# justinmgarrigus/accel-sim-framework-distributed

Measured on AMD Instinct MI355X. Metric: sim KIPS (whole node), higher is better.
Workload: dtype n/a (integer cycle-level model)

## Files before the change

build_native.py:

```python
#!/usr/bin/env python3
from __future__ import annotations

import argparse
import os
import shutil
import subprocess
import sys
import sysconfig

ROOT = os.path.dirname(os.path.abspath(__file__))
PKG = os.path.join(ROOT, "accel_sim_framework_distributed_amd")
ROCM = os.environ.get("ROCM_PATH", "/opt/rocm")
BINARY_PATH_APPS = ("nw", "lud", "hotspot", "backprop", "devcalls")
ARCH = os.environ.get("PYTORCH_ROCM_ARCH", "gfx950")

CORE_SRC = [
    "csrc/config/options.cc",
    "csrc/config/sim_options.cc",
    "csrc/config/icnt_config.cc",
    "csrc/trace/trace.cc",
    "csrc/engine/cpu_engine.cc",
    "csrc/engine/check_engine.cc",
    "csrc/power/power.cc",
    "csrc/power/arch_energy.cc",
    "csrc/driver/simulator.cc",
    "csrc/driver/dump.cc",
    "csrc/driver/debugger.cc",
    "csrc/driver/icnt_bench.cc",
    "csrc/parallel/linksim.cc",
]
HIP_SRC = ["csrc/engine/gpu_engine.hip", "csrc/engine/engine_k_lds.hip", "csrc/engine/engine_k_prof.hip",
           "csrc/engine/engine_k_global.hip", "csrc/engine/engine_k_split.hip", "csrc/engine/engine_k_split2.hip", "csrc/engine/ingest_mfma.hip",
           "csrc/engine/lane_check.hip", "csrc/engine/icnt_sweep.hip"]
STUB_SRC = ["csrc/engine/gpu_stub.cc"]


def _pybind_includes():
    import pybind11
    return [pybind11.get_include(), sysconfig.get_paths()["include"]]


def ext_suffix():
    return sysconfig.get_config_var("EXT_SUFFIX") or ".so"


def have_hipcc():
    return shutil.which("hipcc") is not None or os.path.exists(os.path.join(ROCM, "bin", "hipcc"))


def write_ninja(cpu_only: bool, extra_targets: bool) -> str:
    bdir = os.path.join(ROOT, "build")
    os.makedirs(bdir, exist_ok=True)
    hipcc = shutil.which("hipcc") or os.path.join(ROCM, "bin", "hipcc")
    inc = " ".join(f"-I{p}" for p in [os.path.join(ROOT, "csrc")] + _pybind_includes())
    cxxflags = f"-std=c++17 -O3 -g -fPIC -fopenmp -pthread -Wall -Wno-unused-variable -Wno-unused-function {inc}"
    hipflags = (f"-std=c++17 -O3 -fPIC --offload-arch={ARCH} -munsafe-fp-atomics "
                f"-I{os.path.join(ROOT, 'csrc')}")
    ldflags = f"-fopenmp -pthread -L{ROCM}/lib -Wl,-rpath,{ROCM}/lib"
    lines = [
        "ninja_required_version = 1.3",
        f"cxxflags = {cxxflags}",
        f"hipflags = {hipflags}",
        f"ldflags = {ldflags}",
        "rule cxx",
        "  command = g++ $cxxflags -MMD -MF $out.d -c $in -o $out",
        "  depfile = $out.d",
        "  deps = gcc",
        "  description = CXX $in",
        "rule hip",
        f"  command = {hipcc} $hipflags -MMD -MF $out.d -c $in -o $out",
        "  depfile = $out.d",
        "  deps = gcc",
        "  description = HIP $in",
        "rule link_so",
        "  command = g++ -shared $in -o $out $ldflags $libs",
        "  description = LINK $out",
        "rule link_exe",
        "  command = g++ $in -o $out $ldflags $libs",
        "  description = LINK $out",
        "rule hipexe",
        f"  command = {hipcc} $hipflags $in -o $out $libs",
        "rule isatrace",
        f"  command = {sys.executable} {os.path.join(PKG, 'isatrace', 'build.py')} $in -o $out \"--libs=$libs\" -- "
        f"-munsafe-fp-atomics -fPIC -I{os.path.join(ROOT, 'csrc')}",
        "  description = HIPEXE $out",
        "rule isatrace_bin",
        f"  command = {sys.executable} {os.path.join(PKG, 'isatrace', 'build.py')} $src -o $out --device-from $in "
        f"\"--libs=$libs\" -- -munsafe-fp-atomics -fPIC -I{os.path.join(ROOT, 'csrc')}",
        "  description = HIPEXE-BIN $out",
    ]
    objs = []
    for s in CORE_SRC:
        o = os.path.join(bdir, s.replace("/", "_") + ".o")
        lines.append(f"build {o}: cxx {os.path.join(ROOT, s)}")
        objs.append(o)
    gpu_objs = []
    if not cpu_only:
        for s in HIP_SRC:
            o = os.path.join(bdir, s.replace("/", "_") + ".o")
            lines.append(f"build {o}: hip {os.path.join(ROOT, s)}")
            gpu_objs.append(o)
        libs = "-lamdhip64"
    else:
        for s in STUB_SRC:
            o = os.path.join(bdir, s.replace("/", "_") + ".o")
            lines.append(f"build {o}: cxx {os.path.join(ROOT, s)}")
            gpu_objs.append(o)
        libs = ""
    bind_o = os.path.join(bdir, "bindings.o")
    lines.append(f"build {bind_o}: cxx {os.path.join(ROOT, 'csrc/bindings/py_asim.cc')}")
    main_o = os.path.join(bdir, "main.o")
    lines.append(f"build {main_o}: cxx {os.path.join(ROOT, 'csrc/driver/main.cc')}")
    so = os.path.join(PKG, "_asim" + ext_suffix())
    lines.append(f"build {so}: link_so {' '.join(objs + gpu_objs + [bind_o])}")
    lines.append(f"  libs = {libs}")
# ... 126 lines not shown
```

csrc/bindings/py_asim.cc:

```cpp
#include <chrono>
#include <pybind11/functional.h>
#include <pybind11/numpy.h>
#include <pybind11/pybind11.h>
#include <pybind11/stl.h>

#include <cstring>

#include "../config/icnt_config.h"
#include "../driver/icnt_bench.h"
#include "../driver/simulator.h"
#include "../engine/icnt_sweep.h"

namespace py = pybind11;
using namespace asim;
static const size_t kLinkPktBytes = sizeof(LinkPkt);

namespace {

py::dict link_dict(const LinkParams& p) {
  py::dict d;
  d["link_gbps"] = p.link_gbps;
  d["latency_ns"] = p.latency_ns;
  d["links"] = p.links;
  d["slice_bytes"] = p.slice_bytes;
// ... 533 lines not shown
            if (space != "shared" && space != "global") throw py::value_error("space is 'shared' or 'global'" + at);
            const uint64_t width = py::cast<uint64_t>(t[1]);
            if (width > 255) throw py::value_error("width above 255 bytes per lane" + at);
            const std::string op = py::cast<std::string>(t[4]);
            TInst in{};
            in.cls = OC_LOAD;
            in.space = space == "shared" ? S_SHARED : S_GLOBAL;
            in.width = (uint8_t)width;
            in.mask = py::cast<uint64_t>(t[2]);
            if (!op.empty()) in.opcode = decode_opcode(op, 950).opcode;
            TMem m{};
            if (py::isinstance<py::tuple>(t[3])) {
              const py::tuple bs = py::cast<py::tuple>(t[3]);
              if (bs.size() != 2) throw py::value_error("(base, stride) expected" + at);
              const py::int_ stride = py::cast<py::int_>(bs[1]);
              const long long sv = PyLong_AsLongLong(stride.ptr());
              if (PyErr_Occurred()) {
                PyErr_Clear();
                throw py::value_error("stride outside int32" + at);
              }
              if (sv < INT32_MIN || sv > INT32_MAX) throw py::value_error("stride outside int32" + at);
              m.base = py::cast<uint64_t>(bs[0]);
              m.stride = (int32_t)sv;
              m.list = kNoMem;
            } else {
              const std::vector<uint64_t> a = py::cast<std::vector<uint64_t>>(t[3]);
              if ((size_t)__builtin_popcountll(in.mask) != a.size())
                throw py::value_error("one address per active lane" + at);
              m.list = (uint32_t)k.addrs.size();
              k.addrs.insert(k.addrs.end(), a.begin(), a.end());
              m.base = a.empty() ? 0 : a[0];
            }
            in.mem = (uint32_t)k.mems.size();
            k.mems.push_back(m);
            k.insts.push_back(in);
          }
          k.streams.push_back(WStream{0, (uint32_t)k.insts.size()});
          auto results = [](const ReadyKernel& r) {
            py::list out;
            for (const TInst& in : r.insts) {
              py::list acc;
              if (in.mem != kNoMem)
                for (uint32_t q = 0; q < in.width; ++q) {
                  const TAcc& a = r.accs.at((size_t)in.mem + q);
                  acc.append(py::make_tuple(a.line, (int)a.sectors, (int)a.bytes, (int)a.bank));
                }
              out.append(py::make_tuple(in.space == S_SHARED ? "shared" : "global", (int)in.width, acc));
            }
            return out;
          };
          py::dict d;
          d["host"] = results(coalesce_kernel(k, c));
          d["ran"] = false;
          if (device < 0) return d;
          IngestStats st;
          std::vector<uint8_t> where;
          st.on_device = &where;
          ReadyKernel g;
          if (!gpu_coalesce_kernel(k, c, device, g, &st)) return d;
          d["ran"] = true;
          d["device"] = results(g);
          py::list w;
          for (uint8_t v : where) w.append((int)v);
          d["on_device"] = w;
          d["smem_device"] = st.smem_jobs;
          d["smem_host"] = st.smem_host;
          d["gmem_device"] = st.gmem_jobs;
          d["gmem_host"] = st.gmem_host;
          d["mfma"] = st.mfma;
          return d;
        },
        py::arg("insts"), py::arg("args"), py::arg("device") = -1);
  m.def("lane_policy_check",
        [](const std::string& name, int n, const std::vector<uint64_t>& values, const std::vector<uint64_t>& mask) {
          LaneCheckResult r = lane_policy_check(name, n, values, mask);
          py::dict d;
          d["ran"] = r.ran;
          d["seq"] = r.seq;
          d["stat_words"] = r.stat_words;
          auto bytes_of = [](const std::vector<uint64_t>& v) {
            return py::bytes(reinterpret_cast<const char*>(v.data()), v.size() * 8);
          };
          if (!r.seq_state.empty()) d["seq_state"] = bytes_of(r.seq_state);
          if (r.ran) {
            d["wave"] = r.wave;
            d["stray"] = r.stray;
            if (!r.wave_state.empty()) d["wave_state"] = bytes_of(r.wave_state);
          }
          return d;
        },
        py::arg("case"), py::arg("n"), py::arg("values"), py::arg("mask"));
  m.def("stream_compare", [](const std::string& path, const std::vector<std::string>& args, uint32_t step) {
    SimCfg c = cfg_from_args(args);
    ReadyKernel w = coalesce_kernel(load_kernel_text(path), c);
    ReadyKernel r = open_streamed_kernel(path, c);
    const uint32_t wpc = w.warps_per_cta;
    int64_t bad_cta = -1;
    step = std::max<uint32_t>(1, step);
    for (uint32_t lo = 0; lo < w.n_cta && bad_cta < 0; lo += step) {
      const uint32_t hi = std::min(w.n_cta, lo + step);
      r.resident(lo, hi);
      for (uint32_t cta = lo; cta < hi && bad_cta < 0; ++cta)
        for (uint32_t wi = 0; wi < wpc && bad_cta < 0; ++wi) {
          const WStream& a = w.streams[(size_t)cta * wpc + wi];
          const WStream& b = r.streams[(size_t)(cta - r.cta_lo) * wpc + wi];
          if (a.count != b.count) bad_cta = cta;
          for (uint32_t j = 0; j < a.count && bad_cta < 0; ++j) {
            TInst x = w.insts[a.begin + j];
            TInst y = r.insts[((b.begin + j) - (r.ibase & kStreamInstMask)) & kStreamInstMask];
            const uint32_t xm = x.mem, ym = y.mem;
            x.mem = y.mem = 0;
            if (memcmp(&x, &y, sizeof(TInst)) != 0 || (xm == kNoMem) != (ym == kNoMem)) {
              bad_cta = cta;
              break;
            }
            if (xm == kNoMem) continue;
            const uint64_t yl = (ym - (r.abase & kStreamAccMask)) & kStreamAccMask;
            for (uint32_t q = 0; q < x.width && bad_cta < 0; ++q)
              if (memcmp(&w.accs[xm + q], &r.accs[yl + q], sizeof(TAcc)) != 0) bad_cta = cta;
          }
        }
    }
    py::dict d;
    d["equal"] = bad_cta < 0;
    d["bad_cta"] = bad_cta;
    d["whole_bytes"] = w.host_bytes();
    d["stream_peak_bytes"] = r.host_peak_bytes;
    d["n_cta"] = w.n_cta;
    return d;
  });
  m.def("coalesce_summary", [](const std::string& path, const std::vector<std::string>& args) {
    SimCfg c = cfg_from_args(args);
    ReadyKernel r = coalesce_kernel(load_kernel(path), c);
    py::dict d;
    d["n_accs"] = (uint64_t)r.accs.size();
    uint64_t mem = 0, shared_deg = 0, nshared = 0;
    for (auto& in : r.insts) {
      if (in.mem != kNoMem) mem++;
      if ((in.cls == OC_LOAD || in.cls == OC_STORE) && in.space == S_SHARED) {
        nshared++;
        shared_deg += in.width;
      }
    }
    d["mem_insts"] = mem;
    d["shared_insts"] = nshared;
    d["shared_degree_sum"] = shared_deg;
    py::list acc;
    for (size_t i = 0; i < r.accs.size() && i < 4096; ++i)
      acc.append(py::make_tuple(r.accs[i].line, r.accs[i].sectors, r.accs[i].bytes));
    d["accs"] = acc;
    return d;
  });

  py::class_<Simulator>(m, "Simulator")
      .def(py::init([](const std::vector<std::string>& args, bool echo) {
             py::gil_scoped_release nogil;
             auto* s = new Simulator(args);
             s->set_echo(echo);
             return s;
           }),
           py::arg("args"), py::arg("echo") = false)
      .def("run", &Simulator::run, py::call_guard<py::gil_scoped_release>())
      .def("run_command", &Simulator::run_command, py::call_guard<py::gil_scoped_release>())
      .def("num_commands", [](Simulator& s) { return s.commands().size(); })
      .def("load_commands", &Simulator::load_commands, py::call_guard<py::gil_scoped_release>())
      .def("print_header", [](Simulator& s) { s.load_commands(); })
// ... 171 lines not shown
```

csrc/engine/engine.h:

```cpp
#pragma once
#include <cstring>
#include <memory>
#include <stdexcept>
#include <map>
#include <string>
#include <vector>

#include "../model/epoch.h"
#include "../power/power_eval.h"
#include "../trace/trace.h"

namespace asim {

struct RunLimits {
  uint64_t max_cycle = 0;
  uint64_t max_epochs = 0;
};

struct PwrArm {
  PwrCoef coef;
  uint64_t freq = 0;
  uint64_t t_prev = 0;
  double s_prev[PS_COUNT] = {};
  uint32_t n_sm = 0;
// ... 61 lines not shown
    for (int r = 0; r < PR_COUNT; ++r) {
      const int j = pwr_sum_of(r);
      if (j >= 0) S[j] += (double)pwr_raw_sm(*sm[i], r);
    }
  for (size_t i = 0; i < nmem; ++i)
    for (int r = 0; r < PR_COUNT; ++r) {
      const int j = pwr_sum_of(r);
      if (j >= 0) S[j] += (double)pwr_raw_mem(*mem[i], r);
    }
}

inline PwrSample pwr_take(PwrArm& a, const double* S, uint64_t now) {
  PwrSample o{};
  double d[PS_COUNT];
  for (int j = 0; j < PS_COUNT; ++j) d[j] = S[j] - a.s_prev[j];
  pwr_activity(d, now > a.t_prev ? (double)(now - a.t_prev) : 1.0, a.n_sm, o);
  pwr_power(a.coef, a.coef.coef, a.n_sm, 1.0, 1.0, 1.0, o);
  o.now = now;
  for (int j = 0; j < PS_COUNT; ++j) a.s_prev[j] = S[j];
  a.t_prev = now;
  return o;
}

inline uint32_t backlog_cap(const SimCfg& c) {
  uint64_t b = (uint64_t)c.n_sm * c.icnt_out_limit;
  return (uint32_t)(b < 16384 ? b : 16384);
}

struct EngineStateHeader {
  uint64_t magic = 0x41534d5354415445ull;
  uint64_t version = 8;
  uint64_t n_sm = 0, n_mem = 0, sm_bytes = 0, ch_bytes = 0, pub_bytes = 0;
  uint64_t box_req = 0, cnt_req = 0, box_rep = 0, cnt_rep = 0;
  uint64_t ovf = 0;
  uint64_t mall = 0;
  uint64_t links = 0;
  uint64_t cycle = 0, epoch = 0, ready = 0;
};

struct StateOut {
  std::vector<uint8_t>& v;
  void put(const void* p, size_t n) {
    const size_t o = v.size();
    v.resize(o + n);
    if (n) memcpy(v.data() + o, p, n);
  }
};
struct StateIn {
  const std::vector<uint8_t>& v;
  size_t off = 0;
  const uint8_t* take(size_t n) {
    if (off + n > v.size()) throw std::runtime_error("engine state: truncated image");
    const uint8_t* p = v.data() + off;
    off += n;
    return p;
  }
  void get(void* dst, size_t n) { memcpy(dst, take(n), n); }
};
void check_state_header(const EngineStateHeader& h, const EngineStateHeader& want);

std::unique_ptr<Engine> make_cpu_engine();
std::unique_ptr<Engine> make_gpu_engine();
bool gpu_engine_available();
std::unique_ptr<Engine> make_check_engine(std::unique_ptr<Engine> primary, std::unique_ptr<Engine> reference,
                                          uint64_t interval, uint64_t corrupt_at = 0, bool corrupt_mailbox = false);
int gpu_cu_count();
int gpu_cus_per_sim(uint32_t n_sm, uint32_t n_mem);
std::map<std::string, uint64_t> gpu_pool_stats();
void gpu_pool_trim();
void* gpu_pool_alloc(size_t bytes);
void gpu_pool_release(void* p);
std::map<std::string, uint64_t> gpu_batch_stats();
std::map<std::string, std::map<std::string, uint64_t>> gpu_engine_modes();
struct EngineKernelInfo {
  int num_regs = 0, local_bytes = 0, shared_static = 0, max_threads = 0, binary_version = 0;
  size_t lds_dynamic = 0, sm_state_bytes = 0, chan_state_bytes = 0;
  bool valid = false;
};
EngineKernelInfo gpu_engine_kernel_info();

struct LaneCheckResult {
  std::vector<uint64_t> seq, wave;
  std::vector<uint64_t> seq_state, wave_state;
  bool ran = false;
  bool stray = false;
  uint32_t stat_words = (uint32_t)kStatWords;
};
LaneCheckResult lane_policy_check(const std::string& name, int n, const std::vector<uint64_t>& values,
                                  const std::vector<uint64_t>& mask);

inline uint64_t mall_lines(const SimCfg& c) { return (uint64_t)c.mall_sets * c.mall_assoc; }

uint32_t reply_cap(const SimCfg& c);
void check_core_clock(const SimCfg& c, uint64_t per_core);
void host_memcpy_fill(ChanState* chs, uint32_t nch, const SimCfg& c, uint64_t addr, uint64_t bytes);
void host_flush_l2(ChanState* chs, uint32_t nch, const SimCfg& c, bool writeback = false, L2Line* mall = nullptr);
void init_sm_state(SMState& s, uint32_t id);
void init_chan_state(ChanState& ch, uint32_t id, const SimCfg& c);

}
```

csrc/engine/engine_k_global.hip:

```cpp
#include "engine_kernel.h"

namespace asim {

template __global__ void engine_kernel<WavePar, true, kModeGlobal>(GpuArgs);

__global__ void ASIM_ENGINE_KERNEL_ATTRS engine_batch_kernel(const GpuArgs* __restrict__ jobs,
                                                             const uint16_t* __restrict__ block_job) {
  const uint32_t j = block_job[blockIdx.x];
  const GpuArgs a = jobs[j];
  engine_body<WavePar, true, kModeGlobal>(a, blockIdx.x - a.block0);
}

ASIM_ENGINE_CFG_UPLOAD(global)

}
```

csrc/engine/engine_k_lds.hip:

```cpp
#include "engine_kernel.h"

namespace asim {

template __global__ void engine_kernel<WavePar, false, kModeLds>(GpuArgs);
template __global__ void engine_kernel<WavePar, true, kModeLds>(GpuArgs);

ASIM_ENGINE_CFG_UPLOAD(lds)

}
```

csrc/engine/engine_k_prof.hip:

```cpp
#include "engine_kernel.h"

namespace asim {

template __global__ void engine_kernel<WaveParProf, false, kModeLds>(GpuArgs);
template __global__ void engine_kernel<WaveParProf, true, kModeLds>(GpuArgs);
template __global__ void engine_kernel<WaveParProf, true, kModeGlobal>(GpuArgs);
template __global__ void engine_kernel<WaveParProf, true, kModeSplit>(GpuArgs);

ASIM_ENGINE_CFG_UPLOAD(prof)

}
```

csrc/engine/engine_k_split.hip:

```cpp
#include "engine_kernel.h"

namespace asim {

template __global__ void engine_kernel<WavePar, true, kModeSplit>(GpuArgs);

__global__ void ASIM_ENGINE_KERNEL_ATTRS engine_batch_split_kernel(const GpuArgs* __restrict__ jobs,
                                                                   const uint16_t* __restrict__ block_job) {
  const uint32_t j = block_job[blockIdx.x];
  const GpuArgs a = jobs[j];
  engine_body<WavePar, true, kModeSplit>(a, blockIdx.x - a.block0);
}

ASIM_ENGINE_CFG_UPLOAD(split)

}
```

csrc/engine/engine_k_split2.hip:

```cpp
#include "engine_kernel.h"

namespace asim {

#define ASIM_SPLIT2_KERNEL_ATTRS __launch_bounds__(64) __attribute__((amdgpu_waves_per_eu(2, 2)))

__global__ void ASIM_SPLIT2_KERNEL_ATTRS engine_split2_kernel(GpuArgs a) {
  engine_body<WavePar, true, kModeSplit>(a, blockIdx.x);
}

ASIM_ENGINE_CFG_UPLOAD(split2)

}
```

csrc/engine/engine_kernel.h:

```cpp
#pragma once
#include <hip/hip_runtime.h>

#include "../model/icnt_router_par.h"
#include "engine.h"
#include "grid_barrier.h"
#include "wave_par.h"
#include "sm_split.h"

namespace asim {

constexpr int kCfgSlots = 64;
static __constant__ SimCfg g_cfg[kCfgSlots];

struct PwrDev {
  PwrCoef coef;
  uint64_t freq;
  uint64_t t_prev;
  uint64_t next;
  uint32_t n_sm;
  uint32_t n;
  uint32_t cap;
  uint32_t pad;
  double s_prev[kPwrSumPad];
  double* rows;
// ... 109 lines not shown
template <class T>
__device__ __forceinline__ T* as_global(T* p) {
  typedef __attribute__((address_space(1))) T gT;
  return (T*)(gT*)p;
}

struct WaveParProf : WavePar {
  static __device__ __forceinline__ void prof(int k) {
    ProfLds* p = reinterpret_cast<ProfLds*>(g_lds + kProfOff);
    uint64_t t = __builtin_amdgcn_s_memtime();
    if ((threadIdx.x & 63) == 0) {
      p->acc[p->slot] += t - p->last;
      p->slot = (uint32_t)k;
      p->last = t;
    }
    __builtin_amdgcn_wave_barrier();
  }
  static __device__ __forceinline__ void tick(int k) {
    ProfLds* p = reinterpret_cast<ProfLds*>(g_lds + kProfOff);
    if ((threadIdx.x & 63) == 0) p->acc[k] += 1;
    __builtin_amdgcn_wave_barrier();
  }
};

typedef double f64x4 __attribute__((ext_vector_type(4)));

__device__ __forceinline__ void pwr_row_sm(double* row, const SMStats& st) {
  for (int k = (int)(threadIdx.x & 63); k < kPwrRawPad; k += 64) row[k] = k < PR_COUNT ? (double)pwr_raw_sm(st, k) : 0.0;
}
__device__ __forceinline__ void pwr_row_ch(double* row, const ChanState& ch, uint32_t nsub) {
  for (int k = (int)(threadIdx.x & 63); k < kPwrRawPad; k += 64) {
    double v = 0;
    if (k < PR_COUNT)
      for (uint32_t j = 0; j < nsub; ++j) v += (double)pwr_raw_mem(ch.sp[j].st, k);
    row[k] = v;
  }
}

__device__ void pwr_evaluate(PwrDev& pw, uint32_t nunits, uint64_t now) {
  const int lane = (int)(threadIdx.x & 63);
  constexpr int kCt = kPwrSumPad / 16;
  f64x4 acc[kCt];
#pragma unroll
  for (int ct = 0; ct < kCt; ++ct) acc[ct] = f64x4{0.0, 0.0, 0.0, 0.0};
  const double* rows = pw.rows;
  for (uint32_t t = 0; t < (nunits + 15u) / 16u; ++t) {
    const uint32_t u = 16u * t + (uint32_t)(lane & 15);
    for (int k4 = 0; k4 < kPwrRawPad / 4; ++k4) {
      const int k = 4 * k4 + (lane >> 4);
      const double av = u < nunits ? rows[(size_t)u * kPwrRawPad + k] : 0.0;
      const int sj = k < PR_COUNT ? pwr_sum_of(k) : -1;
#pragma unroll
      for (int ct = 0; ct < kCt; ++ct) {
        const double bv = sj == 16 * ct + (lane & 15) ? 1.0 : 0.0;
        acc[ct] = __builtin_amdgcn_mfma_f64_16x16x4f64(av, bv, acc[ct], 0, 0, 0);
      }
    }
  }
  double* S = reinterpret_cast<double*>(g_lds + kPwrOff);
  double* D = S + kPwrSumPad;
#pragma unroll
  for (int ct = 0; ct < kCt; ++ct) {
    double v = acc[ct][0] + acc[ct][1] + acc[ct][2] + acc[ct][3];
    v += __shfl_xor(v, 16);
    v += __shfl_xor(v, 32);
    if (lane < 16) S[16 * ct + lane] = v;
  }
  __syncthreads();
  if (lane < PS_COUNT) D[lane] = S[lane] - pw.s_prev[lane];
  __syncthreads();
  if (lane == 0) {
    const uint32_t i = pw.n < pw.cap ? pw.n : pw.cap - 1;
    PwrSample& o = pw.ring[i];
    pwr_activity(D, now > pw.t_prev ? (double)(now - pw.t_prev) : 1.0, pw.n_sm, o);
    pwr_power(pw.coef, pw.coef.coef, pw.n_sm, 1.0, 1.0, 1.0, o);
    o.now = now;
    pw.t_prev = now;
    pw.n = pw.n + 1;
  }
  if (lane < PS_COUNT) pw.s_prev[lane] = S[lane];
  __syncthreads();
}

template <class P, bool kSliced, int kMode>
__device__ __forceinline__ void engine_body(const GpuArgs& a, const uint32_t b) {
  constexpr bool kGlobal = kMode == kModeGlobal, kSplit = kMode == kModeSplit;
  const SimCfg& c = g_cfg[a.cfg_slot];
  const uint64_t E = c.icnt_latency;
  SMState* s = reinterpret_cast<SMState*>(g_lds + kStateOff);
  ChanState* ch = reinterpret_cast<ChanState*>(g_lds + kStateOff);
  const uint32_t nunits = c.n_sm + c.n_mem;
  const uint32_t nsmb = a.nblocks - a.ch_blocks;
  auto unit_k = [&](uint32_t k) -> uint32_t {
    if (!a.ch_blocks) return b + k * a.nblocks;
    return b < nsmb ? b + k * nsmb : c.n_sm + (b - nsmb) + k * a.ch_blocks;
  };
  const uint32_t nmine = !kSliced ? 1u
                         : !a.ch_blocks ? (nunits - 1 - b) / a.nblocks + 1
                         : b < nsmb ? (c.n_sm - 1 - b) / nsmb + 1
                                    : (c.n_mem - 1 - (b - nsmb)) / a.ch_blocks + 1;
  const uint32_t u0 = unit_k(0);
  uint32_t loaded = u0;
  auto bind = [&](uint32_t u) {
    if (u < c.n_sm) s = as_global(&a.sms[u]);
    else ch = as_global(&a.chs[u - c.n_sm]);
  };
  uint32_t hot = u0;
  auto swap_to = [&](uint32_t u) {
    if (kGlobal) {
      bind(u);
      loaded = u;
      return;
    }
    if (kSplit) {
      loaded = u;
      if (u >= c.n_sm) {
        ch = as_global(&a.chs[u - c.n_sm]);
        return;
      }
      if (u == hot) return;
      if (hot < c.n_sm) copy_bytes(&a.sms[hot], s, kSmHotBytes);
      copy_bytes(s, &a.sms[u], kSmHotBytes);
      hot = u;
      return;
    }
    if (!kSliced || u == loaded) return;
    if (loaded < c.n_sm) swap_out(&a.sms[loaded], s);
    else swap_out(&a.chs[loaded - c.n_sm], ch);
    if (u < c.n_sm) swap_in(s, &a.sms[u]);
    else swap_in(ch, &a.chs[u - c.n_sm]);
    loaded = u;
  };
  if (kGlobal)
    bind(u0);
  else if (kSplit && u0 < c.n_sm)
    copy_bytes(s, &a.sms[u0], kSmHotBytes);
  else if (kSplit) {
    hot = ~0u;
    ch = as_global(&a.chs[u0 - c.n_sm]);
  } else if (u0 < c.n_sm)
    copy_state(s, &a.sms[u0]);
  else
    copy_state(ch, &a.chs[u0 - c.n_sm]);
  KernelTab* ktl = reinterpret_cast<KernelTab*>(g_lds + kKtOff);
  {
    static_assert(sizeof(KernelTab) % 16 == 0, "kernel table must be 16-byte granular");
    const uint4* src = reinterpret_cast<const uint4*>(a.kt);
    uint4* dst = reinterpret_cast<uint4*>(ktl);
    for (int i = (int)(threadIdx.x & 63); i < (int)(sizeof(KernelTab) / 16); i += 64) dst[i] = src[i];
  }
  ProfLds* pl = reinterpret_cast<ProfLds*>(g_lds + kProfOff);
  if ((threadIdx.x & 63) == 0) {
    pl->last = __builtin_amdgcn_s_memtime();
    pl->slot = 31;
    for (int i = 0; i < kProfSlots; ++i) pl->acc[i] = 0;
  }
  __syncthreads();
  const KernelTab& kt = *ktl;
  SmCtx sx;
  sx.cfg = &c;
  sx.kt = &kt;
  sx.out_cap = a.cap_req;
  sx.n_src_sm = c.n_sm;
  sx.rt_st = c.link_contention == 2 ? a.link_free : nullptr;
  MemCtx mx;
  mx.cfg = &c;
  mx.out_cap = a.cap_rep;
  mx.n_src_sub = c.n_subpart;
  mx.ovf = a.ovf;
  mx.ovf_cap = a.ovf_cap;
  mx.rt_st = c.link_contention == 2 ? a.link_free : nullptr;
  mx.mall = nullptr;
  uint64_t epoch = a.epoch0, cycle = a.cycle0;
  uint64_t t_work0 = a.ework ? __builtin_amdgcn_s_memtime() : 0;
  uint32_t done = 0, dead = 0, capped = 0;
  uint32_t n = 0;
  uint32_t nbar = 0;
  uint64_t pw_next = a.pw ? a.pw->next : 0;
  bool failed = false;
  uint64_t reqm[2] = {~0ull, ~0ull}, repm[2] = {~0ull, ~0ull};
  for (; n < a.max_epochs;) {
    const uint32_t cur = (uint32_t)(epoch & 1), prev = cur ^ 1u;
    const uint64_t t0 = cycle, t1 = t0 + E;
    uint32_t first_k = 0;
    for (uint32_t k = 0; k < nmine; ++k)
      if (unit_k(k) == loaded) first_k = k;
    for (uint32_t j = 0; j < nmine; ++j) {
      const uint32_t u = unit_k((first_k + j) % nmine);
      swap_to(u);
      if (u < c.n_sm) {
        sx.outbox = a.box_req[cur];
        sx.outcnt = a.cnt_req[cur];
        if constexpr (kSplit) {
          SmSplit sp(*s, *as_global(&a.sms[u]));
          sm_epoch<P>(sp, sx, *a.pub, prev, t0, t1, a.box_rep[prev], a.cnt_rep[prev], a.cap_rep, c.n_subpart, epoch,
                      repm);
          sm_publish<P>(sp, sx, *a.pub, cur);
        } else {
          sm_epoch<P>(*s, sx, *a.pub, prev, t0, t1, a.box_rep[prev], a.cnt_rep[prev], a.cap_rep,
                      c.n_subpart, epoch, repm);
          sm_publish<P>(*s, sx, *a.pub, cur);
        }
      } else {
        mx.outbox = a.box_rep[cur];
        mx.outcnt = a.cnt_rep[cur];
        mx.mall = a.mall ? a.mall + (size_t)(u - c.n_sm) * ((size_t)c.mall_sets * c.mall_assoc) : nullptr;
        mx.win_end = core_fs(c, t1);
        chan_epoch<P>(*ch, mx, a.box_req[prev], a.cnt_req[prev], a.cap_req, core_fs(c, t0), reqm);
        chan_publish<P>(*ch, mx, *a.pub, cur);
      }
    }
    ++n;
    P::prof(26);
    uint64_t t_arrive = 0;
    if (a.ework) {
      t_arrive = __builtin_amdgcn_s_memtime();
      if ((threadIdx.x & 63) == 0) a.ework[b] = (uint32_t)(t_arrive - t_work0);
    }
    uint32_t was_last = 0;
    if (!grid_barrier_b(a.ctl, b, a.nblocks, nbar++, &was_last)) break;
    if (a.link_free) {
      const bool rt_par = c.link_contention == 2 && c.router_pass == 1;
      if (rt_par) {
        if (b < 2) {
          const uint32_t dirs = !a.link_refs2 ? (uint32_t)RT_DIR_BOTH : b == 0 ? (uint32_t)RT_DIR_REQ : (uint32_t)RT_DIR_REP;
          const uint32_t rs = rt_epoch_run_par<P>(c, a.box_req[cur], a.cnt_req[cur], a.cap_req, a.box_rep[cur],
                                                  a.cnt_rep[cur], a.cap_rep, a.link_free,
                                                  b == 0 ? a.link_refs : a.link_refs2, dirs, a.rt_pc);
          if (rs != RT_STATUS_OK && (threadIdx.x & 63) == 0)
            __hip_atomic_store(&a.ctl->error, kCtlErrRouterCap, __ATOMIC_RELAXED, __HIP_MEMORY_SCOPE_AGENT);
        }
      } else if (b == 0) {
        icnt_epoch_pass<P>(c, a.box_req[cur], a.cnt_req[cur], a.cap_req, a.box_rep[cur], a.cnt_rep[cur], a.cap_rep,
                           a.link_free, a.link_refs);
      }
      if (!grid_barrier_b(a.ctl, b, a.nblocks, nbar++)) break;
      if (rt_par && P::uni(__hip_atomic_load(&a.ctl->error, __ATOMIC_RELAXED, __HIP_MEMORY_SCOPE_AGENT))) break;
    }
    P::prof(27);
    if (a.ework) {
      const uint64_t t_exit = __builtin_amdgcn_s_memtime();
      if ((threadIdx.x & 63) == 0 && was_last) { pl->acc[34] += t_exit - t_arrive; pl->acc[35] += 1; }
      if (b == 0) {
        uint64_t mk = 0;
        for (uint32_t j = threadIdx.x & 63; j < a.nblocks; j += 64) {
          const uint64_t k = (uint64_t)a.ework[j] << 32 | j;
          mk = k > mk ? k : mk;
        }
        mk = WavePar::red_max64(mk);
        const uint32_t m = (uint32_t)(mk >> 32);
        if ((threadIdx.x & 63) == 0) {
          pl->acc[32] += m;
          pl->acc[33] += 1;
          atomicAdd((unsigned long long*)&a.prof[(size_t)(uint32_t)mk * kProfSlots + 30], 1ull);
        }
      }
      t_work0 = t_exit;
    }
    const uint64_t mc = a.pw ? (a.max_cycle ? (a.max_cycle < pw_next ? a.max_cycle : pw_next) : pw_next) : a.max_cycle;
    EpochDecision d = epoch_decide<P>(c, *a.pub, cur, t1, kt, epoch, mc);
    reqm[0] = P::uni(d.req_dst[0]);
    reqm[1] = P::uni(d.req_dst[1]);
    repm[0] = P::uni(d.rep_dst[0]);
    repm[1] = P::uni(d.rep_dst[1]);
    P::prof(28);
    ++epoch;
    cycle = P::uni(d.next_start);
    if (a.pw) {
      const bool exits = P::uni(d.done) || P::uni(d.deadlock) || P::uni(d.limit) || (a.max_cycle && cycle >= a.max_cycle);
      if (exits || cycle >= pw_next) {
        for (uint32_t k = 0; k < nmine; ++k) {
          const uint32_t u = unit_k(k);
          double* row = a.pw->rows + (size_t)u * kPwrRawPad;
          if (u < c.n_sm) pwr_row_sm(row, (!kGlobal && u == (kSplit ? hot : loaded)) ? s->st : a.sms[u].st);
          else pwr_row_ch(row, (!kGlobal && !kSplit && u == loaded) ? *ch : a.chs[u - c.n_sm], c.n_sub_per_mem);
        }
        if (!grid_barrier_b(a.ctl, b, a.nblocks, nbar++)) { failed = true; break; }
        if (b == a.nblocks - 1) pwr_evaluate(*a.pw, nunits, cycle);
        pw_next = cycle + a.pw->freq;
      }
    }
    if (P::uni(d.done)) { done = P::uni(d.done); break; }
    if (P::uni(d.deadlock)) { dead = 1; break; }
    if (P::uni(d.limit)) { capped = 1; break; }
    if (P::uni(d.refill)) break;
    if (a.max_cycle && cycle >= a.max_cycle) break;
  }
  P::prof(31);
  if (kGlobal)
    ;
  else if (kSplit) {
    if (hot < c.n_sm) copy_bytes(&a.sms[hot], s, kSmHotBytes);
  } else if (loaded < c.n_sm)
    copy_state(&a.sms[loaded], s);
  else
    copy_state(&a.chs[loaded - c.n_sm], ch);
  if (a.prof && (threadIdx.x & 63) < kProfSlots && (threadIdx.x & 63) != 30) a.prof[(size_t)b * kProfSlots + (threadIdx.x & 63)] += pl->acc[threadIdx.x & 63];
  (void)failed;
  if (a.pw && b == 0 && (threadIdx.x & 63) == 0) a.pw->next = pw_next;
  if (b == 0 && (threadIdx.x & 63) == 0) {
    a.ctl->done = done;
    a.ctl->deadlock = dead;
    a.ctl->cap = capped;
    a.ctl->end_cycle = cycle;
    a.ctl->end_epoch = epoch;
    a.ctl->epochs_run = n;
  }
}


#define ASIM_ENGINE_KERNEL_ATTRS __launch_bounds__(64) __attribute__((amdgpu_waves_per_eu(1, 1)))

template <class P, bool kSliced, int kMode>
__global__ void ASIM_ENGINE_KERNEL_ATTRS engine_kernel(GpuArgs a) {
  engine_body<P, kSliced, kMode>(a, blockIdx.x);
}

__global__ void ASIM_ENGINE_KERNEL_ATTRS engine_batch_kernel(const GpuArgs* __restrict__ jobs,
                                                             const uint16_t* __restrict__ block_job);
__global__ void ASIM_ENGINE_KERNEL_ATTRS engine_batch_split_kernel(const GpuArgs* __restrict__ jobs,
                                                                   const uint16_t* __restrict__ block_job);

__global__ void engine_split2_kernel(GpuArgs a);

#define ASIM_ENGINE_CFG_UPLOAD(name)                                                         \
  hipError_t engine_upload_cfg_##name(const SimCfg& c, int slot) {                          \
    return hipMemcpyToSymbol(HIP_SYMBOL(g_cfg), &c, sizeof(SimCfg), sizeof(SimCfg) * (size_t)slot, \
                             hipMemcpyHostToDevice);                                         \
  }

}
```

csrc/engine/gpu_engine.hip:

```cpp
#include <hip/hip_runtime.h>

#include <algorithm>
#include <cerrno>
#include <csignal>
#include <cstdio>
#include <cstring>
#include <map>
#include <memory>
#include <stdexcept>
#include <string>

#include <fcntl.h>
#include <sys/file.h>
#include <sys/stat.h>
#include <unistd.h>
#include <chrono>
#include <condition_variable>
#include <deque>
#include <mutex>
#include <vector>

#include "engine_kernel.h"
#include "trace_window.h"

namespace asim {

#define HIPCHECK(x)                                                                                  \
  do {                                                                                               \
    hipError_t e_ = (x);                                                                             \
    if (e_ != hipSuccess)                                                                            \
      throw std::runtime_error(std::string("HIP error: ") + hipGetErrorString(e_) + " at " #x);    \
  } while (0)

extern template __global__ void engine_kernel<WavePar, false, kModeLds>(GpuArgs);
extern template __global__ void engine_kernel<WavePar, true, kModeLds>(GpuArgs);
extern template __global__ void engine_kernel<WaveParProf, false, kModeLds>(GpuArgs);
extern template __global__ void engine_kernel<WaveParProf, true, kModeLds>(GpuArgs);
extern template __global__ void engine_kernel<WavePar, true, kModeGlobal>(GpuArgs);
extern template __global__ void engine_kernel<WaveParProf, true, kModeGlobal>(GpuArgs);
extern template __global__ void engine_kernel<WavePar, true, kModeSplit>(GpuArgs);
extern template __global__ void engine_kernel<WaveParProf, true, kModeSplit>(GpuArgs);
hipError_t engine_upload_cfg_lds(const SimCfg& c, int slot);
hipError_t engine_upload_cfg_prof(const SimCfg& c, int slot);
hipError_t engine_upload_cfg_global(const SimCfg& c, int slot);
hipError_t engine_upload_cfg_split(const SimCfg& c, int slot);
hipError_t engine_upload_cfg_split2(const SimCfg& c, int slot);

namespace {

class DeviceCuTable {
 public:
  struct Ent {
    int32_t pid;
    int32_t cus;
  };
  static constexpr int kMax = 256;
  explicit DeviceCuTable(int dev) {
    char bus[64] = {0};
    if (hipDeviceGetPCIBusId(bus, sizeof(bus), dev) != hipSuccess) snprintf(bus, sizeof(bus), "dev%d", dev);
    for (char* q = bus; *q; ++q)
      if (*q == ':' || *q == '.') *q = '_';
    path_ = std::string("/tmp/asim_gpu_cus_") + bus + ".lock";
    fd_ = open(path_.c_str(), O_RDWR | O_CREAT, 0666);
    if (fd_ >= 0) (void)fchmod(fd_, 0666);
  }
  ~DeviceCuTable() {
    if (fd_ >= 0) close(fd_);
  }
  void acquire(int n, int cap) {
    if (fd_ < 0) return;
    for (int spin = 0;; ++spin) {
      if (flock(fd_, LOCK_EX) != 0) return;
      std::vector<Ent> e = load();
      int used = 0;
      for (const Ent& x : e) used += x.cus;
      if (used + n <= cap || e.empty()) {
        e.push_back(Ent{(int32_t)getpid(), (int32_t)n});
        store(e);
        flock(fd_, LOCK_UN);
        return;
      }
      flock(fd_, LOCK_UN);
      usleep(spin < 100 ? 200 : 2000);
    }
  }
  void release(int n) {
    if (fd_ < 0 || flock(fd_, LOCK_EX) != 0) return;
    std::vector<Ent> e = load();
    for (size_t i = 0; i < e.size(); ++i)
      if (e[i].pid == (int32_t)getpid() && e[i].cus == n) {
        e.erase(e.begin() + (long)i);
        break;
      }
    store(e);
    flock(fd_, LOCK_UN);
  }

 private:
  std::vector<Ent> load() {
    std::vector<Ent> e(kMax);
    const ssize_t r = pread(fd_, e.data(), sizeof(Ent) * kMax, 0);
    e.resize(r > 0 ? (size_t)r / sizeof(Ent) : 0);
    std::vector<Ent> live;
    for (const Ent& x : e)
      if (x.pid > 0 && x.cus > 0 && (kill(x.pid, 0) == 0 || errno == EPERM)) live.push_back(x);
    return live;
  }
  void store(const std::vector<Ent>& e) {
    if (ftruncate(fd_, 0) != 0) return;
    if (!e.empty()) (void)pwrite(fd_, e.data(), sizeof(Ent) * e.size(), 0);
  }
  std::string path_;
  int fd_ = -1;
};

constexpr uint32_t kCuSlots = 840;
constexpr uint32_t kMaxBlocksPerCu = 8;
uint32_t block_slots(size_t lds) {
  const size_t per_cu = lds ? (160 * 1024) / lds : kMaxBlocksPerCu;
  return kCuSlots / (uint32_t)std::max<size_t>(1, std::min<size_t>(per_cu, kMaxBlocksPerCu));
}
int gpu_state_mode() {
  const char* e = getenv("ASIM_GPU_STATE");
  if (!e || !*e) return kModeSplit;
  const std::string v(e);
  return v == "global" ? kModeGlobal : v == "lds" ? kModeLds : kModeSplit;
}
bool gpu_state_global() { return gpu_state_mode() == kModeGlobal; }
int split_waves() {
  const char* e = getenv("ASIM_GPU_SPLIT_WAVES");
  return e && atoi(e) == 2 ? 2 : 1;
}
int g_occ_api = 0;
uint32_t mode_blocks_per_cu(int mode) {
  if (mode == kModeLds) return 1;
  static std::mutex mu;
  static uint32_t cache[3] = {0, 0, 0};
  std::lock_guard<std::mutex> g(mu);
  if (!cache[mode]) {
    int occ = 0;
    const void* f = mode == kModeGlobal ? (const void*)engine_batch_kernel
                    : split_waves() == 2 ? (const void*)engine_split2_kernel
                                         : (const void*)engine_kernel<WavePar, true, kModeSplit>;
    const size_t lds = mode == kModeGlobal ? kLdsBytesGlobal : kLdsBytesSplit;
    if (hipOccupancyMaxActiveBlocksPerMultiprocessor(&occ, f, 64, (int)lds) != hipSuccess) occ = 2;
    g_occ_api = occ;
    occ = occ > 1 ? occ - 1 : 1;
    if (const char* e = getenv("ASIM_GPU_BLOCKS_PER_CU"))
      if (atoi(e) > 0) occ = atoi(e);
    cache[mode] = (uint32_t)std::min<int>(occ, (int)kMaxBlocksPerCu);
  }
  return cache[mode];
}
uint32_t global_blocks_per_cu() { return mode_blocks_per_cu(kModeGlobal); }
struct BlockPlan {
  uint32_t nblocks, ch_blocks;
};
BlockPlan block_plan(uint32_t n_sm, uint32_t n_mem, int mode, uint32_t cap) {
  BlockPlan p{n_sm + n_mem, 0};
  if (mode == kModeSplit && n_sm > 0 && n_mem > 0) {
    uint32_t pack = 1;
    if (const char* e = getenv("ASIM_GPU_CH_PER_BLOCK"))
      if (atoi(e) > 0) pack = (uint32_t)atoi(e);
    const uint32_t chb = (n_mem + pack - 1) / pack;
    if (pack > 1 && n_sm + chb <= cap) p = BlockPlan{n_sm + chb, chb};
  }
  if (p.nblocks > cap) p = BlockPlan{cap, 0};
  return p;
}
uint32_t engine_block_slots(int mode) { return kCuSlots / mode_blocks_per_cu(mode); }
bool profiling_env() {
  const char* pe = getenv("ASIM_GPU_PROFILE");
  return pe && *pe && *pe != '0';
}
bool gpu_batch_on() {
  const char* e = getenv("ASIM_GPU_BATCH");
  return e && std::string(e) == "1";
}

class CuPool {
 public:
  static CuPool& get() {
    static CuPool p;
    return p;
  }
  void init(int cus) {
    std::lock_guard<std::mutex> g(mu_);
    if (cap_ == 0) {
      cap_ = free_ = cus;
      int dev = 0;
      if (hipGetDevice(&dev) == hipSuccess) table_.reset(new DeviceCuTable(dev));
    }
  }
  void acquire(int n) {
    {
      std::unique_lock<std::mutex> g(mu_);
      cv_.wait(g, [&] { return free_ >= n; });
      free_ -= n;
    }
    if (table_) table_->acquire(n, cap_);
  }
  void release(int n) {
    if (table_) table_->release(n);
    {
      std::lock_guard<std::mutex> g(mu_);
      free_ += n;
    }
    cv_.notify_all();
  }
  int capacity() {
    std::lock_guard<std::mutex> g(mu_);
    return cap_;
  }

 private:
  std::mutex mu_;
  std::condition_variable cv_;
  int cap_ = 0, free_ = 0;
  std::unique_ptr<DeviceCuTable> table_;
};

class CfgSlots {
 public:
  static CfgSlots& get() {
    static CfgSlots s;
    return s;
// ... 279 lines not shown
      if (e == hipSuccess) e = hipMalloc(&sl.d_bj, sizeof(uint16_t) * nbk);
      if (e == hipSuccess) e = hipHostMalloc(&sl.h_jobs, sizeof(GpuArgs) * nj);
      if (e == hipSuccess) e = hipHostMalloc(&sl.h_bj, sizeof(uint16_t) * nbk);
      if (e != hipSuccess) {
        sl.jobs_cap = sl.blocks_cap = 0;
        return e;
      }
      sl.jobs_cap = nj;
      sl.blocks_cap = nbk;
    }
    uint32_t b0 = 0;
    for (size_t j = 0; j < njobs; ++j) {
      GpuArgs a = take[j]->a;
      a.block0 = b0;
      sl.h_jobs[j] = a;
      for (uint32_t i = 0; i < take[j]->nb; ++i) sl.h_bj[b0 + i] = (uint16_t)j;
      b0 += take[j]->nb;
    }
    hipError_t e = hipMemcpyAsync(sl.d_jobs, sl.h_jobs, sizeof(GpuArgs) * njobs, hipMemcpyHostToDevice, sl.stream);
    if (e == hipSuccess) e = hipMemcpyAsync(sl.d_bj, sl.h_bj, sizeof(uint16_t) * blocks, hipMemcpyHostToDevice, sl.stream);
    for (size_t j = 0; j < njobs && e == hipSuccess; ++j) e = hipMemsetAsync(take[j]->a.ctl, 0, sizeof(GpuCtl), sl.stream);
    if (e != hipSuccess) return e;
    CuPool::get().acquire((int)slots);
    if (mode == kModeSplit)
      hipLaunchKernelGGL(engine_batch_split_kernel, dim3(blocks), dim3(64), kLdsBytesSplit, sl.stream,
                         (const GpuArgs*)sl.d_jobs, (const uint16_t*)sl.d_bj);
    else
      hipLaunchKernelGGL(engine_batch_kernel, dim3(blocks), dim3(64), kLdsBytesGlobal, sl.stream,
                         (const GpuArgs*)sl.d_jobs, (const uint16_t*)sl.d_bj);
    e = hipGetLastError();
    for (size_t j = 0; j < njobs; ++j) {
      const hipError_t ce =
          hipMemcpyAsync(take[j]->h_ctl, take[j]->a.ctl, sizeof(GpuCtl), hipMemcpyDeviceToHost, sl.stream);
      if (e == hipSuccess) e = ce;
    }
    const hipError_t se = hipStreamSynchronize(sl.stream);
    CuPool::get().release((int)slots);
    return e != hipSuccess ? e : se;
  }

  std::mutex mu_;
  std::condition_variable cv_;
  std::deque<Sub*> pending_;
  std::chrono::steady_clock::time_point first_;
  int running_ = 0;
  int in_flight_ = 0;
  int in_run_ = 0;
  Slot slots_[kMaxBatches];
  uint64_t batches_ = 0, jobs_ = 0;
};

class GpuEngine : public Engine {
 public:
  ~GpuEngine() override {
    try {
      dump_profile();
    } catch (...) {
    }
    DevicePool::get().dev_free(d_prof_);
    DevicePool::get().dev_free(d_ework_);
    release();
    if (cfg_slot_ >= 0) CfgSlots::get().release(cfg_slot_);
  }
  const char* name() const override { return "gpu"; }

  void init(const SimCfg& c) override {
    c_ = c;
    int dev = 0;
    HIPCHECK(hipGetDevice(&dev));
    hipDeviceProp_t prop;
    HIPCHECK(hipGetDeviceProperties(&prop, dev));
    n_cu_ = prop.multiProcessorCount;
    CuPool::get().init(n_cu_ * kCuSlots);
    mode_ = gpu_state_mode();
    uint32_t cap = (uint32_t)n_cu_ * mode_blocks_per_cu(mode_);
    if (const char* eb = getenv("ASIM_GPU_BLOCKS"))
      if (atoi(eb) > 0) cap = std::min<uint32_t>(cap, (uint32_t)atoi(eb));
    const BlockPlan bp = block_plan(c.n_sm, c.n_mem, mode_, cap);
    nblocks_ = bp.nblocks;
    ch_blocks_ = bp.ch_blocks;
    global_ = mode_ == kModeGlobal;
    lds_ = global_ ? kLdsBytesGlobal : mode_ == kModeSplit ? kLdsBytesSplit : kLdsBytes;
    sliced_ = nblocks_ < c.n_sm + c.n_mem;
    for (const void* f : {(const void*)engine_kernel<WavePar, false, kModeLds>, (const void*)engine_kernel<WaveParProf, false, kModeLds>,
                          (const void*)engine_kernel<WavePar, true, kModeLds>, (const void*)engine_kernel<WaveParProf, true, kModeLds>})
      HIPCHECK(hipFuncSetAttribute(f, hipFuncAttributeMaxDynamicSharedMemorySize, (int)kLdsBytes));
    slots_ = engine_block_slots(mode_);
    batch_ = (global_ || mode_ == kModeSplit) && !profiling_env() && gpu_batch_on();
    if (cfg_slot_ < 0) cfg_slot_ = CfgSlots::get().acquire();
    const char* pe = getenv("ASIM_GPU_PROFILE");
    profiling_ = pe && *pe && *pe != '0';
    if (profiling_) {
      pool_alloc(&d_prof_, sizeof(uint64_t) * nblocks_ * kProfSlots);
      HIPCHECK(hipMemset(d_prof_, 0, sizeof(uint64_t) * nblocks_ * kProfSlots));
      pool_alloc(&d_ework_, sizeof(uint32_t) * nblocks_);
    }
    stream_ = DevicePool::get().stream();
    if (!done_ev_) HIPCHECK(hipEventCreateWithFlags(&done_ev_, hipEventBlockingSync | hipEventDisableTiming));
    if (c_.trace_mask) {
      const size_t units = (size_t)c.n_sm + c.n_mem;
      pool_alloc(&d_trace_ev_, units * c_.trace_cap * sizeof(TraceEv));
      pool_alloc(&d_trace_cnt_, units * sizeof(uint32_t));
      HIPCHECK(hipMemset(d_trace_cnt_, 0, units * sizeof(uint32_t)));
      c_.trace_ev = d_trace_ev_;
      c_.trace_cnt = d_trace_cnt_;
    }
    pool_alloc(&d_cfg_, sizeof(SimCfg));
    upload_cfg();
    std::vector<SMState> hs(c.n_sm);
    for (uint32_t i = 0; i < c.n_sm; ++i) init_sm_state(hs[i], i);
    std::vector<ChanState> hc(c.n_mem);
    for (uint32_t i = 0; i < c.n_mem; ++i) init_chan_state(hc[i], i, c);
    pool_alloc(&d_sms_, sizeof(SMState) * c.n_sm);
    pool_alloc(&d_chs_, sizeof(ChanState) * c.n_mem);
    HIPCHECK(hipMemcpy(d_sms_, hs.data(), sizeof(SMState) * c.n_sm, hipMemcpyHostToDevice));
    HIPCHECK(hipMemcpy(d_chs_, hc.data(), sizeof(ChanState) * c.n_mem, hipMemcpyHostToDevice));
    pool_alloc(&d_pub_, sizeof(EpochPub));
    HIPCHECK(hipMemset(d_pub_, 0, sizeof(EpochPub)));
    cap_req_ = c.icnt_latency;
    cap_rep_ = reply_cap(c);
    for (int p = 0; p < 2; ++p) {
      pool_alloc(&d_box_req_[p], sizeof(Pkt) * c.n_subpart * c.n_sm * cap_req_);
      HIPCHECK(hipMemset(d_box_req_[p], 0, sizeof(Pkt) * c.n_subpart * c.n_sm * cap_req_));
      pool_alloc(&d_cnt_req_[p], sizeof(uint32_t) * c.n_subpart * c.n_sm);
      HIPCHECK(hipMemset(d_cnt_req_[p], 0, sizeof(uint32_t) * c.n_subpart * c.n_sm));
      pool_alloc(&d_box_rep_[p], sizeof(Pkt) * c.n_sm * c.n_subpart * cap_rep_);
      HIPCHECK(hipMemset(d_box_rep_[p], 0, sizeof(Pkt) * c.n_sm * c.n_subpart * cap_rep_));
      pool_alloc(&d_cnt_rep_[p], sizeof(uint32_t) * c.n_sm * c.n_subpart);
      HIPCHECK(hipMemset(d_cnt_rep_[p], 0, sizeof(uint32_t) * c.n_sm * c.n_subpart));
    }
    ovf_cap_ = backlog_cap(c);
    pool_alloc(&d_ovf_, sizeof(Pkt) * c.n_subpart * (size_t)ovf_cap_);
    HIPCHECK(hipMemset(d_ovf_, 0, sizeof(Pkt) * c.n_subpart * (size_t)ovf_cap_));
    n_mall_ = (size_t)c.n_mem * mall_lines(c);
    if (n_mall_) {
      pool_alloc(&d_mall_, sizeof(L2Line) * n_mall_);
      HIPCHECK(hipMemset(d_mall_, 0, sizeof(L2Line) * n_mall_));
    }
    if (c.link_contention && (icnt_link_count(c) > kMaxIcntLinks || !icnt_contention_fits(c, cap_req_, cap_rep_) ||
                              icnt_scratch_words(c, cap_req_, cap_rep_) > kMaxIcntScratchWords))
      throw std::runtime_error("-icnt_link_contention: topology or mailboxes too large for the link pass");
    n_links_ = icnt_contention_on(c) ? (size_t)icnt_state_words(c, cap_req_, cap_rep_) : 0;
    if (n_links_) {
      pool_alloc(&d_links_, sizeof(uint64_t) * (n_links_ + kIcntStatWords));
      HIPCHECK(hipMemset(d_links_, 0, sizeof(uint64_t) * (n_links_ + kIcntStatWords)));
      pool_alloc(&d_link_refs_, sizeof(uint32_t) * (size_t)icnt_scratch_words(c, cap_req_, cap_rep_));
      if (router_par()) {
        if (nblocks_ >= 2) pool_alloc(&d_link_refs2_, sizeof(uint32_t) * (size_t)icnt_scratch_words(c, cap_req_, cap_rep_));
        pool_alloc(&d_rt_pc_, sizeof(RtPassCount));
        HIPCHECK(hipMemset(d_rt_pc_, 0, sizeof(RtPassCount)));
      }
    }
    pool_alloc(&d_ctl_, sizeof(GpuCtl));
    h_ctl_ = static_cast<GpuCtl*>(DevicePool::get().host(sizeof(GpuCtl)));
    pool_alloc(&d_kt_, sizeof(KernelTab));
    kt_ = KernelTab{};
    kt_.mix = c.concurrent_kernel_sm;
    epoch_ = 0;
    cycle_ = 0;
  }

  void launch(uint32_t slot, ReadyKernel& k, const KernelDesc& kd) override {
    if (slot >= (uint32_t)kMaxConc || (kt_.active >> slot & 1u)) throw std::runtime_error("launch: kernel slot busy");
    if (!k.streamed() && k.insts.size() > kIdxMask) throw std::runtime_error("kernel trace exceeds 2^29 warp instructions");
    KernelDesc& d = kt_.k[slot];
    d = kd;
    tw_.launch(slot, k, d, c_);
    kt_.active |= 1u << slot;
  }
  uint32_t running() const override { return kt_.active; }

  RunResult run(const RunLimits& lim) override {
    RunResult res;
    if (!kt_.active) {
      res.end_cycle = cycle_;
      return res;
    }
    struct InRun {
      bool on;
      explicit InRun(bool b) : on(b) {
        if (on) BatchLauncher::get().enter();
      }
      ~InRun() {
        if (on) BatchLauncher::get().leave();
      }
    } in_run(batch_);
    for (;;) {
      tw_.ensure(kt_, c_, [&](DispatchView& v) { read_dispatch(v); });
      HIPCHECK(hipMemcpy(d_kt_, &kt_, sizeof(KernelTab), hipMemcpyHostToDevice));
      GpuArgs a{};
      a.cfg_slot = (uint32_t)cfg_slot_;
      a.cfg_g = d_cfg_;
      a.kt = d_kt_;
      a.sms = d_sms_;
      a.chs = d_chs_;
      a.pub = d_pub_;
      for (int p = 0; p < 2; ++p) {
        a.box_req[p] = d_box_req_[p];
        a.cnt_req[p] = d_cnt_req_[p];
        a.box_rep[p] = d_box_rep_[p];
        a.cnt_rep[p] = d_cnt_rep_[p];
      }
      a.cap_req = cap_req_;
      a.cap_rep = cap_rep_;
      a.ovf = d_ovf_;
      a.ovf_cap = ovf_cap_;
      a.mall = d_mall_;
      a.link_free = d_links_;
      a.link_refs = d_link_refs_;
      a.link_refs2 = d_link_refs2_;
      a.rt_pc = d_rt_pc_;
      a.epoch0 = epoch_;
      a.cycle0 = cycle_;
      a.max_cycle = lim.max_cycle;
      a.max_epochs = epochs_per_launch_;
      a.nblocks = nblocks_;
      a.ch_blocks = ch_blocks_;
      a.ctl = d_ctl_;
      HIPCHECK(hipMemsetAsync(d_ctl_, 0, sizeof(GpuCtl), stream_));
      a.prof = d_prof_;
      a.ework = d_ework_;
      a.pw = pw_on_ ? d_pw_ : nullptr;
      if (batch_) {
        a.max_epochs = std::min<uint32_t>(a.max_epochs, BatchLauncher::kBatchEpochs);
        BatchLauncher::Sub sub;
        sub.a = a;
        sub.mode = mode_;
        sub.nb = nblocks_;
        sub.slots = slots_;
        sub.h_ctl = h_ctl_;
        variant_ = "batch";
        BatchLauncher::get().run(sub);
        ++launches_;
        HIPCHECK(sub.err);
      } else {
      CuPool::get().acquire((int)(nblocks_ * slots_));
      hipError_t le;
      if (mode_ == kModeSplit && profiling_) {
        variant_ = "split_prof";
        hipLaunchKernelGGL((engine_kernel<WaveParProf, true, kModeSplit>), dim3(nblocks_), dim3(64), lds_, stream_, a);
      } else if (mode_ == kModeSplit && split_waves() == 2) {
        variant_ = "split2";
        hipLaunchKernelGGL(engine_split2_kernel, dim3(nblocks_), dim3(64), lds_, stream_, a);
      } else if (mode_ == kModeSplit) {
        variant_ = "split";
        hipLaunchKernelGGL((engine_kernel<WavePar, true, kModeSplit>), dim3(nblocks_), dim3(64), lds_, stream_, a);
      } else if (global_ && profiling_) {
        variant_ = "global_prof";
        hipLaunchKernelGGL((engine_kernel<WaveParProf, true, kModeGlobal>), dim3(nblocks_), dim3(64), lds_, stream_, a);
      } else if (global_) {
        variant_ = "global";
        hipLaunchKernelGGL((engine_kernel<WavePar, true, kModeGlobal>), dim3(nblocks_), dim3(64), lds_, stream_, a);
      } else if (profiling_ && sliced_) {
        variant_ = "lds_sliced_prof";
        hipLaunchKernelGGL((engine_kernel<WaveParProf, true, kModeLds>), dim3(nblocks_), dim3(64), lds_, stream_, a);
      } else if (profiling_) {
        variant_ = "lds_prof";
        hipLaunchKernelGGL((engine_kernel<WaveParProf, false, kModeLds>), dim3(nblocks_), dim3(64), lds_, stream_, a);
      } else if (sliced_) {
        variant_ = "lds_sliced";
        hipLaunchKernelGGL((engine_kernel<WavePar, true, kModeLds>), dim3(nblocks_), dim3(64), lds_, stream_, a);
      } else {
        variant_ = "lds";
        hipLaunchKernelGGL((engine_kernel<WavePar, false, kModeLds>), dim3(nblocks_), dim3(64), lds_, stream_, a);
      }
      le = hipGetLastError();
      ++launches_;
      hipError_t ce = hipMemcpyAsync(h_ctl_, d_ctl_, sizeof(GpuCtl), hipMemcpyDeviceToHost, stream_);
      hipError_t se = hipEventRecord(done_ev_, stream_);
      if (se == hipSuccess) se = hipEventSynchronize(done_ev_);
      CuPool::get().release((int)(nblocks_ * slots_));
      HIPCHECK(le);
      HIPCHECK(ce);
      HIPCHECK(se);
      }
      if (h_ctl_->error == kCtlErrRouterCap) throw std::runtime_error(kRouterStepCapMsg);
      if (h_ctl_->error) throw std::runtime_error("GPU engine: grid barrier timed out (blocks not co-resident?)");
      epoch_ = h_ctl_->end_epoch;
      cycle_ = h_ctl_->end_cycle;
      if (pw_on_) pwr_collect();
      res.epochs += h_ctl_->epochs_run;
      if (h_ctl_->done) {
        res.done = true;
        res.done_mask = h_ctl_->done;
        kt_.active &= ~h_ctl_->done;
        for (uint32_t s = 0; s < (uint32_t)kMaxConc; ++s)
          if (h_ctl_->done >> s & 1u) tw_.done(s);
        break;
      }
      if (h_ctl_->deadlock) { res.deadlock = true; break; }
      if (h_ctl_->cap) { res.hit_limit = true; res.cap = true; break; }
      if ((lim.max_cycle && cycle_ >= lim.max_cycle) || (lim.max_epochs && res.epochs >= lim.max_epochs)) {
        res.hit_limit = true;
        break;
      }
      if (h_ctl_->epochs_run == 0) throw std::runtime_error("GPU engine made no progress");
    }
    res.end_cycle = cycle_;
    return res;
  }

  uint64_t now() const override { return cycle_; }

  void memcpy_fill_l2(uint64_t addr, uint64_t bytes) override {
    std::vector<ChanState> hc(c_.n_mem);
    HIPCHECK(hipMemcpy(hc.data(), d_chs_, sizeof(ChanState) * c_.n_mem, hipMemcpyDeviceToHost));
    host_memcpy_fill(hc.data(), c_.n_mem, c_, addr, bytes);
    HIPCHECK(hipMemcpy(d_chs_, hc.data(), sizeof(ChanState) * c_.n_mem, hipMemcpyHostToDevice));
  }
  void set_core_clock(uint64_t per_core, uint64_t base_cyc, uint64_t base_fs) override {
    check_core_clock(c_, per_core);
    c_.per_core = per_core;
    c_.clk_base_cyc = base_cyc;
    c_.clk_base_fs = base_fs;
    cfg_set_divs(c_);
    upload_cfg();
  }
  void flush_l2(bool writeback) override {
    std::vector<ChanState> hc(c_.n_mem);
    HIPCHECK(hipMemcpy(hc.data(), d_chs_, sizeof(ChanState) * c_.n_mem, hipMemcpyDeviceToHost));
    std::vector<L2Line> hm(writeback ? n_mall_ : 0);
    if (!hm.empty()) HIPCHECK(hipMemcpy(hm.data(), d_mall_, sizeof(L2Line) * n_mall_, hipMemcpyDeviceToHost));
    host_flush_l2(hc.data(), c_.n_mem, c_, writeback, hm.empty() ? nullptr : hm.data());
    HIPCHECK(hipMemcpy(d_chs_, hc.data(), sizeof(ChanState) * c_.n_mem, hipMemcpyHostToDevice));
    if (!hm.empty()) HIPCHECK(hipMemcpy(d_mall_, hm.data(), sizeof(L2Line) * n_mall_, hipMemcpyHostToDevice));
  }

  void stats(std::vector<SMStats>& sm, std::vector<MemStats>& mem) override {
    sm.resize(c_.n_sm);
    HIPCHECK(hipMemcpy2D(sm.data(), sizeof(SMStats), reinterpret_cast<char*>(d_sms_) + offsetof(SMState, st),
                         sizeof(SMState), sizeof(SMStats), c_.n_sm, hipMemcpyDeviceToHost));
    mem.clear();
    for (uint32_t j = 0; j < c_.n_sub_per_mem; ++j) {
      std::vector<MemStats> part(c_.n_mem);
      size_t off = offsetof(ChanState, sp) + j * sizeof(SubPart) + offsetof(SubPart, st);
      HIPCHECK(hipMemcpy2D(part.data(), sizeof(MemStats), reinterpret_cast<char*>(d_chs_) + off, sizeof(ChanState),
                           sizeof(MemStats), c_.n_mem, hipMemcpyDeviceToHost));
      if (j == 0) mem.resize((size_t)c_.n_mem * c_.n_sub_per_mem);
      for (uint32_t i = 0; i < c_.n_mem; ++i) mem[(size_t)i * c_.n_sub_per_mem + j] = part[i];
    }
  }

  void snapshot(std::vector<uint8_t>& out) override {
    const size_t units = sizeof(SMState) * c_.n_sm + sizeof(ChanState) * c_.n_mem;
    out.resize(units + sizeof(L2Line) * n_mall_ + 8 * n_links_);
    HIPCHECK(hipMemcpy(out.data(), d_sms_, sizeof(SMState) * c_.n_sm, hipMemcpyDeviceToHost));
    HIPCHECK(hipMemcpy(out.data() + sizeof(SMState) * c_.n_sm, d_chs_, sizeof(ChanState) * c_.n_mem,
                       hipMemcpyDeviceToHost));
    if (n_mall_) HIPCHECK(hipMemcpy(out.data() + units, d_mall_, sizeof(L2Line) * n_mall_, hipMemcpyDeviceToHost));
// ... 118 lines not shown
    cycle_ = h.cycle;
    epoch_ = h.epoch;
    if (h.ready) throw std::runtime_error("engine state: image taken with kernels running");
  }

 private:
  void pwr_collect() {
    uint32_t n = 0;
    HIPCHECK(hipMemcpy(&n, reinterpret_cast<char*>(d_pw_) + offsetof(PwrDev, n), sizeof(n), hipMemcpyDeviceToHost));
    if (n > pw_cap_) throw std::runtime_error("GPU engine: power sample ring overflow");
    if (n) {
      const size_t o = pw_out_.size();
      pw_out_.resize(o + n);
      HIPCHECK(hipMemcpy(pw_out_.data() + o, d_pw_ring_, sizeof(PwrSample) * n, hipMemcpyDeviceToHost));
      const uint32_t z = 0;
      HIPCHECK(hipMemcpy(reinterpret_cast<char*>(d_pw_) + offsetof(PwrDev, n), &z, sizeof(z), hipMemcpyHostToDevice));
    }
  }

  void read_dispatch(DispatchView& v) {
    const size_t off_d = offsetof(SMState, k_uid);
    const size_t len_d = offsetof(SMState, next_ctax) + sizeof(SMState::next_ctax) - off_d;
    std::vector<char> disp(len_d);
    HIPCHECK(hipMemcpy(disp.data(), reinterpret_cast<char*>(d_sms_) + off_d, len_d, hipMemcpyDeviceToHost));
    memcpy(v.k_uid, disp.data() + (offsetof(SMState, k_uid) - off_d), sizeof(v.k_uid));
    memcpy(v.next_cta, disp.data() + (offsetof(SMState, next_cta) - off_d), sizeof(v.next_cta));
    memcpy(v.next_ctax, disp.data() + (offsetof(SMState, next_ctax) - off_d), sizeof(v.next_ctax));
    const size_t off_c = offsetof(SMState, cta_id);
    const size_t len_c = offsetof(SMState, cta_wbase) - off_c;
    std::vector<char> ctas((size_t)c_.n_sm * len_c);
    HIPCHECK(hipMemcpy2D(ctas.data(), len_c, reinterpret_cast<char*>(d_sms_) + off_c, sizeof(SMState), len_c, c_.n_sm,
                         hipMemcpyDeviceToHost));
    v.sms.resize(c_.n_sm);
    for (uint32_t m = 0; m < c_.n_sm; ++m) {
      const char* e = ctas.data() + (size_t)m * len_c;
      memcpy(v.sms[m].cta_id, e, sizeof(v.sms[m].cta_id));
      memcpy(v.sms[m].cta_valid, e + (offsetof(SMState, cta_valid) - off_c), sizeof(v.sms[m].cta_valid));
      memcpy(v.sms[m].cta_ks, e + (offsetof(SMState, cta_ks) - off_c), sizeof(v.sms[m].cta_ks));
    }
  }

 public:
  void trace_residency(uint64_t* peak_bytes, uint64_t* refills) const override {
    *peak_bytes = tw_.resident_peak;
    *refills = tw_.refills;
  }

  uint64_t launches() const override { return launches_; }
  const char* kernel_variant() const override { return variant_; }
  uint32_t kernel_blocks() const override { return *variant_ ? nblocks_ : 0; }
  bool power_sampler() const override { return true; }
  void power_arm(const PwrArm& arm) override {
    const uint32_t nunits = c_.n_sm + c_.n_mem;
    const uint32_t cap = epochs_per_launch_ + 2;
    if (!d_pw_) pool_alloc(&d_pw_, sizeof(PwrDev));
    if (!d_pw_rows_) pool_alloc(&d_pw_rows_, sizeof(double) * kPwrRawPad * nunits);
    if (pw_cap_ < cap) {
      DevicePool::get().dev_free(d_pw_ring_);
      pool_alloc(&d_pw_ring_, sizeof(PwrSample) * cap);
      pw_cap_ = cap;
    }
    PwrDev h{};
    h.coef = arm.coef;
    h.freq = arm.freq;
    h.t_prev = arm.t_prev;
    h.next = arm.t_prev + arm.freq;
    h.n_sm = arm.n_sm;
    h.n = 0;
    h.cap = pw_cap_;
    for (int j = 0; j < PS_COUNT; ++j) h.s_prev[j] = arm.s_prev[j];
    h.rows = d_pw_rows_;
    h.ring = d_pw_ring_;
    HIPCHECK(hipMemcpy(d_pw_, &h, sizeof(PwrDev), hipMemcpyHostToDevice));
    pw_on_ = true;
    pw_out_.clear();
  }
  void power_disarm() override { pw_on_ = false; }
  void power_drain(std::vector<PwrSample>& out) override {
    out.swap(pw_out_);
    pw_out_.clear();
  }

 private:
  void upload_cfg() {
    HIPCHECK(hipMemcpy(d_cfg_, &c_, sizeof(SimCfg), hipMemcpyHostToDevice));
    HIPCHECK(engine_upload_cfg_lds(c_, cfg_slot_));
    HIPCHECK(engine_upload_cfg_prof(c_, cfg_slot_));
    HIPCHECK(engine_upload_cfg_global(c_, cfg_slot_));
    HIPCHECK(engine_upload_cfg_split(c_, cfg_slot_));
    HIPCHECK(engine_upload_cfg_split2(c_, cfg_slot_));
  }
  void release() {
    auto fr = [](void* p) {
      DevicePool::get().dev_free(p);
    };
    fr(d_cfg_);
    fr(d_sms_);
    fr(d_chs_);
    fr(d_pub_);
    for (int p = 0; p < 2; ++p) {
      fr(d_box_req_[p]);
      fr(d_cnt_req_[p]);
      fr(d_box_rep_[p]);
      fr(d_cnt_rep_[p]);
    }
    fr(d_ctl_);
    fr(d_ovf_);
    fr(d_mall_);
    fr(d_links_);
    fr(d_link_refs_);
    fr(d_link_refs2_);
    fr(d_rt_pc_);
    d_link_refs2_ = nullptr;
    d_rt_pc_ = nullptr;
    n_links_ = 0;
    fr(d_trace_ev_);
    fr(d_trace_cnt_);
    tw_.release();
    fr(d_pw_);
    fr(d_pw_rows_);
    fr(d_pw_ring_);
    fr(d_kt_);
    DevicePool::get().host_free(h_ctl_);
    DevicePool::get().stream_free(stream_);
    if (done_ev_) (void)hipEventDestroy(done_ev_);
    done_ev_ = nullptr;
  }

  SimCfg c_{};
  int cfg_slot_ = -1;
  int n_cu_ = 0;
  uint32_t nblocks_ = 0;
  uint32_t ch_blocks_ = 0;
  size_t lds_ = 0;
  hipStream_t stream_ = nullptr;
  hipEvent_t done_ev_ = nullptr;
  SimCfg* d_cfg_ = nullptr;
  SMState* d_sms_ = nullptr;
  ChanState* d_chs_ = nullptr;
  EpochPub* d_pub_ = nullptr;
  Pkt* d_ovf_ = nullptr;
  L2Line* d_mall_ = nullptr;
  size_t n_mall_ = 0;
  uint64_t* d_links_ = nullptr;
  uint32_t* d_link_refs_ = nullptr;
  uint32_t* d_link_refs2_ = nullptr;
  RtPassCount* d_rt_pc_ = nullptr;
  size_t n_links_ = 0;
  uint32_t ovf_cap_ = 0;
  Pkt* d_box_req_[2] = {nullptr, nullptr};
  uint32_t* d_cnt_req_[2] = {nullptr, nullptr};
  Pkt* d_box_rep_[2] = {nullptr, nullptr};
  uint32_t* d_cnt_rep_[2] = {nullptr, nullptr};
  GpuCtl* d_ctl_ = nullptr;
  GpuCtl* h_ctl_ = nullptr;
  TraceEv* d_trace_ev_ = nullptr;
  uint32_t* d_trace_cnt_ = nullptr;
  struct DevMem {
    static constexpr bool kHost = false;
    void* alloc(size_t n) {
      void* p = nullptr;
      pool_alloc(&p, n);
      return p;
    }
    void free(void* p) {
      DevicePool::get().dev_free(p);
    }
    void write(void* d, const void* h, size_t n) { HIPCHECK(hipMemcpy(d, h, n, hipMemcpyHostToDevice)); }
  };
  TraceWindows<DevMem> tw_;
  uint64_t launches_ = 0;
  const char* variant_ = "";
  bool pw_on_ = false;
// ... 52 lines not shown
        n_ep += (double)h[(size_t)b * kProfSlots + 19];
      }
      fprintf(stderr, "[asim gpu profile] SM cycles simulated %.0f (%.0f clocks each), quiet checks %.0f "
                      "(cycle_loop %.0f clocks each), busy SM-epochs %.0f\n",
              n_cyc, n_cyc ? cyc_clk / n_cyc : 0, n_q, n_q ? q_clk / n_q : 0, n_ep);
    }
    {
      double mx = 0, ne = 0, lw = 0, nl = 0;
      for (uint32_t b = 0; b < nblocks_; ++b) {
        mx += (double)h[(size_t)b * kProfSlots + 32];
        ne += (double)h[(size_t)b * kProfSlots + 33];
        lw += (double)h[(size_t)b * kProfSlots + 34];
        nl += (double)h[(size_t)b * kProfSlots + 35];
      }
      fprintf(stderr, "[asim gpu profile] epochs %.0f: slowest block's work %.0f clocks/epoch; last arriver's "
                      "barrier wait %.0f clocks/epoch (pure barrier latency)\n",
              ne, ne ? mx / ne : 0, nl ? lw / nl : 0);
    }
    {
      std::vector<std::pair<uint64_t, uint32_t>> sl;
      for (uint32_t b = 0; b < nblocks_; ++b) sl.push_back({h[(size_t)b * kProfSlots + 30], b});
      std::sort(sl.rbegin(), sl.rend());
      fprintf(stderr, "[asim gpu profile] slowest block per epoch (epochs, block, its SM cycles / quiet checks):");
      for (size_t i = 0; i < sl.size() && i < 8 && sl[i].first; ++i)
        fprintf(stderr, " %llu x b%u (%s, %llu/%llu)", (unsigned long long)sl[i].first, sl[i].second,
                sl[i].second < c_.n_sm ? "SM" : "MEM", (unsigned long long)h[(size_t)sl[i].second * kProfSlots + 17],
                (unsigned long long)h[(size_t)sl[i].second * kProfSlots + 18]);
      fprintf(stderr, "\n");
    }
    uint32_t crit = 0;
    double crit_work = -1;
    for (uint32_t b = 0; b < nblocks_; ++b) {
      double w = 0;
      for (int k = 0; k < kProfSlots; ++k)
        if (k != 26 && k != 30 && !(k >= 17 && k <= 19) && !(k >= 32 && k <= 35)) w += (double)h[(size_t)b * kProfSlots + k];
      if (w > crit_work) { crit_work = w; crit = b; }
    }
    fprintf(stderr, "[asim gpu profile] shader-clock cycles per block (mean), share of block time; "
                    "CRIT = block %u (%s), the one with the least barrier wait\n", crit, crit < c_.n_sm ? "SM" : "MEM");
    double ct = 0;
    for (int k = 0; k < kProfSlots; ++k)
      if (k != 30 && !(k >= 17 && k <= 19) && !(k >= 32 && k <= 35)) ct += (double)h[(size_t)crit * kProfSlots + k];
    for (int k = 0; k < kProfSlots; ++k) {
      const double cv = (double)h[(size_t)crit * kProfSlots + k];
      if (sm[k] + mc[k] > 0)
        fprintf(stderr, "  %-18s SM %14.0f (%5.1f%%)   MEM %14.0f (%5.1f%%)   CRIT %14.0f (%5.1f%%)\n", names[k], sm[k],
                100 * sm[k] / smt, mc[k], 100 * mc[k] / mct, cv, 100 * cv / ct);
    }
  }

};

}

bool gpu_engine_available() {
  int n = 0;
  if (hipGetDeviceCount(&n) != hipSuccess) return false;
  return n > 0;
}

std::unique_ptr<Engine> make_gpu_engine() {
  if (!gpu_engine_available()) return nullptr;
  return std::unique_ptr<Engine>(new GpuEngine());
}

}

namespace asim {
std::map<std::string, uint64_t> gpu_pool_stats() {
  const DevicePool::Stats t = DevicePool::get().stats();
  return {{"cached_dev", t.cached_dev}, {"cached_host", t.cached_host}, {"cap_dev", t.cap_dev},
          {"cap_host", t.cap_host}, {"trims", t.trims}, {"freed_over_cap", t.freed_over_cap}};
}
void gpu_pool_trim() { DevicePool::get().trim(); }
void* gpu_pool_alloc(size_t bytes) { return DevicePool::get().dev(bytes); }
void gpu_pool_release(void* p) { DevicePool::get().dev_free(p); }
std::map<std::string, std::map<std::string, uint64_t>> gpu_engine_modes() {
  std::map<std::string, std::map<std::string, uint64_t>> out;
  const struct {
    const char* name;
    int mode;
    const void* f;
    size_t lds;
  } ms[] = {{"lds", kModeLds, (const void*)engine_kernel<WavePar, false, kModeLds>, kLdsBytes},
            {"global", kModeGlobal, (const void*)engine_batch_kernel, kLdsBytesGlobal},
            {"split", kModeSplit, (const void*)engine_kernel<WavePar, true, kModeSplit>, kLdsBytesSplit},
            {"split2", kModeSplit, (const void*)engine_split2_kernel, kLdsBytesSplit}};
  for (const auto& m : ms) {
    auto& o = out[m.name];
    o["lds_bytes"] = m.lds;
    o["blocks_per_cu"] = mode_blocks_per_cu(m.mode);
    int occ = 0;
    if (m.mode == kModeLds) (void)hipFuncSetAttribute(m.f, hipFuncAttributeMaxDynamicSharedMemorySize, (int)kLdsBytes);
    if (hipOccupancyMaxActiveBlocksPerMultiprocessor(&occ, m.f, 64, (int)m.lds) == hipSuccess) o["occupancy_api"] = occ;
    hipFuncAttributes fa;
    if (hipFuncGetAttributes(&fa, m.f) == hipSuccess) {
      o["num_regs"] = (uint64_t)fa.numRegs;
      o["scratch_bytes_per_lane"] = (uint64_t)fa.localSizeBytes;
    }
  }
  out["split"]["sm_hot_bytes"] = kSmHotBytes;
  out["lds"]["sm_state_bytes"] = sizeof(SMState);
  return out;
}
std::map<std::string, uint64_t> gpu_batch_stats() {
  std::map<std::string, uint64_t> m{{"batches", BatchLauncher::get().batches()},
                                     {"launches", BatchLauncher::get().jobs()},
                                     {"blocks_per_cu", global_blocks_per_cu()},
                                     {"occupancy_api", (uint64_t)g_occ_api}};
  hipFuncAttributes fa;
  if (hipFuncGetAttributes(&fa, (const void*)engine_batch_kernel) == hipSuccess) {
    m["num_regs"] = (uint64_t)fa.numRegs;
    m["scratch_bytes_per_lane"] = (uint64_t)fa.localSizeBytes;
  }
  return m;
}
int gpu_cus_per_sim(uint32_t n_sm, uint32_t n_mem) {
  const int m = gpu_state_mode();
  const int cus = gpu_cu_count();
  uint32_t cap = cus > 0 ? (uint32_t)cus * mode_blocks_per_cu(m) : n_sm + n_mem;
  if (const char* eb = getenv("ASIM_GPU_BLOCKS"))
    if (atoi(eb) > 0) cap = std::min<uint32_t>(cap, (uint32_t)atoi(eb));
  const uint32_t nb = block_plan(n_sm, n_mem, m, cap).nblocks;
  const uint32_t slots = nb * engine_block_slots(m);
  return (int)((slots + kCuSlots - 1) / kCuSlots);
}
int gpu_cu_count() {
  int dev = 0;
  if (hipGetDevice(&dev) != hipSuccess) return 0;
  hipDeviceProp_t p;
  if (hipGetDeviceProperties(&p, dev) != hipSuccess) return 0;
  return p.multiProcessorCount;
}
}

namespace asim {
EngineKernelInfo gpu_engine_kernel_info() {
  EngineKernelInfo k;
  hipFuncAttributes fa;
  if (hipFuncGetAttributes(&fa, (const void*)engine_kernel<WavePar, false, kModeLds>) != hipSuccess) return k;
  k.num_regs = fa.numRegs;
  k.local_bytes = (int)fa.localSizeBytes;
  k.shared_static = (int)fa.sharedSizeBytes;
  k.max_threads = fa.maxThreadsPerBlock;
  k.binary_version = fa.binaryVersion;
  k.lds_dynamic = kLdsBytes;
  k.sm_state_bytes = sizeof(SMState);
  k.chan_state_bytes = sizeof(ChanState);
  k.valid = true;
  return k;
}
}
```

csrc/engine/lane_check.h:

```cpp
#pragma once
#include <cstdint>
#include <cstring>
#include <stdexcept>
#include <string>
#include <vector>

#include "../model/hd.h"
#include "../model/sm.h"
#include "engine.h"

namespace asim {

enum LaneCase : int {
  LC_BALLOT = 0, LC_BALLOT_M, LC_EACH_M, LC_RED_SUM, LC_RED_OR, LC_SUM, LC_VMAX, LC_VOR, LC_RED_SUM64, LC_RED_MIN64,
  LC_RED_MAX64, LC_ARGMIN, LC_FIND_FIRST, LC_SCAN, LC_ORDER16, LC_LANES, LC_UNI, LC_FETCH, LC_REG, LC_SB, LC_STAT,
  LC_VIEW, LC_MIN32
};

constexpr int kLaneScratch = 1024;
constexpr uint8_t kLaneCanary = 0xEE;
constexpr int kLaneMaxN = 4096;

struct LaneArgs {
  int id, sub, n;
  const uint64_t* val;
  int nval;
  const uint64_t* m;
  int nm;
  uint64_t* out;
  uint8_t* scratch;
};

struct LanePlan {
  int id = 0, sub = 0;
  size_t nout = 0;
  bool state = false;
  bool split = false;
  bool scratch_hbm = false;
};

template <class T>
SIM_HDI T lane_mk(uint64_t v) {
  const uint64_t w[2] = {v, ~v};
  T r;
  __builtin_memcpy(&r, w, sizeof(T));
  return r;
}
template <class T>
SIM_HDI void lane_emit(const T& x, uint64_t* o) {
  uint64_t w[2] = {0, 0};
  __builtin_memcpy(w, &x, sizeof(T));
  o[0] = w[0];
  o[1] = w[1];
}
struct LaneB16 { uint32_t w[4]; };
struct LaneB32 { uint32_t w[8]; };

template <class P, class T, int N>
struct LaneReg {
  T (&a)[N];
  SIM_HDI explicit LaneReg(T (&arr)[N]) : a(arr) {}
  SIM_HDI T& operator[](int w) { return a[w]; }
  SIM_HDI void store(T (&)[N]) {}
};

template <class P, class T>
SIM_HD void lane_lanes_case(const LaneArgs& a) {
  auto L = P::template lanes<T>(a.n, [&](int i) { return lane_mk<T>(a.val[i]); });
  uint64_t* o = a.out;
  for (int k = 0; k < a.nm; ++k) {
    const T x = L.at((int)a.m[k]);
    P::one([&] { lane_emit(x, o + 2 * k); });
  }
  o += 2 * a.nm;
  P::each(a.n, [&](int i) { lane_emit(L.self(i), o + 2 * i); });
}

template <class P, class T>
SIM_HD void lane_uni_case(const LaneArgs& a) {
  const T x = P::uni(lane_mk<T>(a.val[0]));
  P::one([&] { lane_emit(x, a.out); });
}

template <class P, class T>
SIM_HD void lane_fetch_case(const LaneArgs& a) {
  P::fetch_copy(reinterpret_cast<T*>(a.scratch), reinterpret_cast<const T*>(a.val), a.n);
  P::fetch_wait();
  P::sync();
  const uint64_t* s = reinterpret_cast<const uint64_t*>(a.scratch);
  P::each(kLaneScratch / 8, [&](int i) { a.out[i] = s[i]; });
}

template <class P, class T, int N>
SIM_HD void lane_reg_case(const LaneArgs& a) {
  T(&all)[64] = *reinterpret_cast<T(*)[64]>(a.scratch);
  P::each(64, [&](int i) { all[i] = (T)a.val[i]; });
  P::sync();
  T(&arr)[N] = *reinterpret_cast<T(*)[N]>(a.scratch);
  LaneReg<P, T, N> r(arr);
  const uint64_t live = N >= 64 ? ~0ull : ((1ull << (N & 63)) - 1);
  uint64_t* o = a.out;
  for (int k = 0; k < a.nm; ++k) {
    const T x = r[(int)a.m[k]];
    P::one([&] { o[k] = (uint64_t)(int64_t)x; });
  }
  o += a.nm;
  P::each_m(live, [&](int i) { o[i] = (uint64_t)(int64_t)(T)r[i]; });
  o += 64;
  for (int k = 0; k < a.nm; ++k) P::each_m(1ull << a.m[k], [&](int i) { o[k] = (uint64_t)(int64_t)(T)r[i]; });
  o += a.nm;
  for (int k = 0; k < a.nm; ++k) {
    const int j = (int)a.m[k];
    const T x = (T)a.val[64 + k];
// ... 212 lines not shown

template <class P, class S>
SIM_HD void lane_view_case(const LaneArgs& a, S& s) {
  const bool upd = a.val[1] != 0;
  const uint64_t mk = a.m[0];
  P::view(s, [&](auto& v) {
    if (!upd) return;
    v.last_progress = 0x1122334455667788ull;
    v.epoch_end += 3;
    v.age_ctr += 7;
    v.n_cta_active = 5;
    v.live_mask ^= 0x8000000000000001ull;
    v.fetch_rr += 1;
    v.n_pend = 9;
    v.idoc_mask |= 1ull << 40;
    v.oc_mask &= 0x0f0fu;
    v.l1_stamp += 2;
    v.skipped_cycles += 11;
    v.min_emit = ~0ull;
    v.outq_head = 3;
    v.outq_n += 1;
    v.outstanding += 2;
    v.inq_head = 1;
    v.inq_n += 4;
    v.cl_head = 2;
    v.cl_n += 1;
    v.ld_head = 1;
    v.ld_n += 1;
    v.cycle += 1;
    v.arb_next = 3;
    v.used_thr += 64;
    v.ldst.busy = 1;
    v.ldst.warp = 17;
    v.ldst.start += 5;
    v.ldst.inst.pc = 0x1230;
    v.ldst.inst.mask = 0xf0f0f0f0f0f0f0f0ull;
    v.w_next[0] = 77;
    v.w_next[63] += 1;
    v.w_end[5] = v.w_next[0];
    v.w_flags[63] |= 0x80;
    v.w_ibuf[1] += 2;
    v.w_cta[62] = 31;
    v.w_inflight[7]++;
    v.w_stores[0] += 3;
    v.w_loads[63] -= 1;
    v.w_slot_used[9] |= 0x11;
    v.idoc_meta[kIdOc - 1] = idoc_pack(3, 2, 1);
    v.oc_info[kMaxOC - 1] += 1ull << 32;
    v.oc_banks[0] = 0xffff0102030405ull;
    v.oc_age[3] = 99;
    v.fu_next[U_COUNT * kMaxSched - 1] += 4;
    v.wb_occ[0] |= 1ull << 63;
    v.hit_occ[0] &= ~1ull;
    v.cta_valid[kMaxCta - 1] = 1;
    v.cta_live[0]--;
    v.cta_bar[5] += 1;
    v.cta_nexit[kMaxCta - 1] = 2;
    v.sched_last[kMaxSched - 1] = 9;
    v.w_iline[17] = 0xabcdef0123456789ull;
    v.w_wait[4] = 0x0102;
    v.cta_id[2] = 1234;
    v.wb_cnt[3] += 1;
    v.l1[2].lru = 5;
    P::each_m(mk, [&](int w) {
      v.w_head[w] += (uint32_t)w;
      v.w_age[w] = v.w_next[w];
      v.w_flags[w] &= 0x7f;
    });
    sbs(v.w_sb, 3, 1);
    sbs(v.w_sb, 3, 255);
    sbc(v.w_sb, 9, 64);
    sbz(v.w_sb, 12);
    P::each_m(mk, [&](int w) { sbs(v.w_sb, (uint32_t)w, (uint8_t)(4 * w + 1)); });
    v.sadd(0, 5);
    v.sadd(63, 1);
    v.sadd(64, 1ull << 40);
    v.sadd((uint32_t)kStatWords - 1, 3);
    v.template sadd_r<kLaneStatLo, kLaneStatHi>(64, 2);
    v.sset(130, v.sget(63) + 1);
  });
}

template <class P, class S>
SIM_HD void lane_case_state(const LaneArgs& a, S& s) {
  if (a.id == LC_SB) lane_sb_case<P>(a, s);
  else if (a.id == LC_STAT) lane_stat_case<P>(a, s);
  else lane_view_case<P>(a, s);
}


inline void lane_fill_pattern(std::vector<uint64_t>& img, uint64_t seed) {
  uint64_t x = seed;
  for (auto& w : img) {
    x += 0x9e3779b97f4a7c15ull;
    uint64_t z = x;
    z = (z ^ (z >> 30)) * 0xbf58476d1ce4e5b9ull;
    z = (z ^ (z >> 27)) * 0x94d049bb133111ebull;
    w = z ^ (z >> 31);
  }
}

inline LanePlan lane_plan(const std::string& name, int n, const std::vector<uint64_t>& val,
                          const std::vector<uint64_t>& m) {
  auto bad = [&](const char* why) { throw std::invalid_argument("lane_policy_check(" + name + "): " + why); };
  auto need = [&](bool ok, const char* why) {
    if (!ok) bad(why);
  };
  LanePlan p;
  const size_t nv = val.size(), nm = m.size();
  need(nv < (1u << 20) && nm < (1u << 20), "input too long");
  static const char* simple[] = {"ballot", "ballot_m", "each_m", "red_sum", "red_or", "sum", "vmax", "vor",
                                 "red_sum64", "red_min64", "red_max64", "argmin", "find_first", "scan", "order16"};
  for (int i = 0; i < 15; ++i)
    if (name == simple[i]) {
      p.id = i;
      p.nout = 1;
      if (i == LC_BALLOT) need(n >= 0 && n <= 64 && nv >= (size_t)n, "n <= 64 values");
      else if (i == LC_BALLOT_M || i == LC_EACH_M) {
        need(nv >= 64 && nm >= 1, "64 values and a mask");
        if (i == LC_EACH_M) p.nout = 64;
      } else if (i == LC_ORDER16) {
        need(n >= 0 && n <= 16 && nv >= (size_t)n && nm >= 1, "n <= 16 keys and a mask");
        need((m[0] >> n) == 0, "mask bits must be below n");
      } else {
        need(n >= 0 && n <= kLaneMaxN && nv >= (size_t)n, "n values, n <= 4096");
        if (i == LC_SCAN) p.nout = (size_t)n + 1;
      }
      return p;
    }
  if (name == "min32") {
    need(n >= 0 && n <= kLaneMaxN && nv >= (size_t)n && nm >= (size_t)n, "n values and n slots, n <= 4096");
    for (int i = 0; i < n; ++i) need(m[i] < 64, "slot below 64");
    p.id = LC_MIN32;
    p.nout = 64;
    return p;
  }
  auto tail_int = [&](const std::string& prefix) -> int {
    if (name.compare(0, prefix.size(), prefix) != 0) return -1;
    const std::string t = name.substr(prefix.size());
    if (t.empty() || t.size() > 3 || t.find_first_not_of("0123456789") != std::string::npos) return -1;
    return atoi(t.c_str());
  };
  int k;
  if ((k = tail_int("lanes")) >= 0) {
    need(k == 4 || k == 8 || k == 16, "lanes4 / lanes8 / lanes16");
    need(n >= 0 && n <= 64 && nv >= (size_t)n, "n <= 64 values");
    for (uint64_t i : m) need(i < (uint64_t)n, "lane index must be below n");
    p.id = LC_LANES;
    p.sub = k;
    p.nout = 2 * nm + 128;
    return p;
  }
  if ((k = tail_int("uni")) >= 0) {
    need(k == 1 || k == 2 || k == 4 || k == 8 || k == 16, "uni1 / 2 / 4 / 8 / 16");
    need(nv >= 1, "one value");
    p.id = LC_UNI;
    p.sub = k;
    p.nout = 2;
    return p;
  }
  for (const char* pre : {"fetch_lds", "fetch_hbm"})
    if ((k = tail_int(pre)) >= 0) {
      need(k == 16 || k == 32, "16- or 32-byte records");
      need(n >= 1 && n * (k / 16) <= 64, "1 record up to 64 16-byte chunks");
      need(nv >= (size_t)n * (k / 8), "n records of values");
      p.id = LC_FETCH;
      p.sub = k;
      p.scratch_hbm = std::string(pre) == "fetch_hbm";
      p.nout = kLaneScratch / 8;
      return p;
    }
  if (name.compare(0, 4, "reg_") == 0) {
    static const char* types[] = {"u8", "i8", "u16", "i16", "u32", "i32", "u64", "i64"};
    static const int extents[] = {16, 48, 64};
    for (int t = 0; t < 8; ++t)
      for (int e = 0; e < 3; ++e)
        if (name == std::string("reg_") + types[t] + "_" + std::to_string(extents[e])) {
          need(nm >= 1 && nm <= 64 && nv >= 64 + nm, "64 values, then one per index");
          for (uint64_t i : m) need(i < (uint64_t)extents[e], "index must be below the extent");
          p.id = LC_REG;
          p.sub = t << 2 | e;
          p.nout = 3 * nm + 128;
          return p;
        }
    bad("unknown register type / extent");
  }
  if (name == "sb" || name == "stat" || name == "view") {
    p.state = true;
    need(n == 0 || n == 1, "n: 0 = SMState, 1 = SmSplit");
    p.split = n == 1;
    need(nm <= 4096, "at most 4096 operations");
    if (name == "sb") {
      p.id = LC_SB;
      need(nv >= 193, "3 x 64 registers and the state seed");
      for (size_t i = 0; i < 192; ++i) need(val[i] < 256, "register below 256");
      for (uint64_t o : m) need((o & 0xff) < 4 && (o >> 8 & 0xff) < 64 && (o >> 24) == 0, "op < 4, warp < 64, register < 256");
      p.nout = nm + 1 + 256;
    } else if (name == "stat") {
      p.id = LC_STAT;
      need(nv >= 1 && nm % 2 == 0, "the state seed; (op | counter << 8, operand) pairs");
      for (size_t i = 0; i < nm; i += 2) {
        const uint64_t op = m[i] & 0xff, c = m[i] >> 8;
        need(op < 6 && c < (uint64_t)kStatWords, "op < 6, counter below kStatWords");
        if (op == 1) need(c < 64, "sadd_r<0, 64>: counter below 64");
        if (op == 2) need(c >= kLaneStatLo && c < kLaneStatHi, "sadd_r<60, 70>: counter in [60, 70)");
      }
      p.nout = nm / 2 + (size_t)kStatWords;
    } else {
      p.id = LC_VIEW;
      need(nv >= 2 && nm >= 1, "seed, update flag; a warp mask");
      p.nout = 0;
    }
    return p;
  }
  bad("unknown case");
  return p;
}

inline uint64_t lane_state_seed(const LanePlan& p, const std::vector<uint64_t>& val) {
  return val[p.id == LC_SB ? 192 : 0];
}

inline void lane_check_host(const LanePlan& p, int n, const std::vector<uint64_t>& val, const std::vector<uint64_t>& m,
                            LaneCheckResult& r) {
  r.seq.assign(p.nout, 0);
  alignas(16) uint8_t scratch[kLaneScratch];
  memset(scratch, kLaneCanary, sizeof(scratch));
  std::vector<uint64_t> vbuf(val.size() + 2);
  uint64_t* v = vbuf.data();
  if (reinterpret_cast<uintptr_t>(v) % 16) ++v;
  if (!val.empty()) memcpy(v, val.data(), val.size() * 8);
  LaneArgs a{p.id, p.sub, n, v, (int)val.size(), m.data(), (int)m.size(), r.seq.data(), scratch};
  if (!p.state) {
    lane_case_prim<SeqPar>(a);
    return;
  }
  static_assert(sizeof(SMState) % 16 == 0, "SMState is a whole number of 16-byte words");
  const size_t words = sizeof(SMState) / 8;
  r.seq_state.assign(words, 0);
  lane_fill_pattern(r.seq_state, lane_state_seed(p, val));
  std::vector<uint64_t> al(words + 2);
  uint64_t* ap = al.data();
  if (reinterpret_cast<uintptr_t>(ap) % 16) ++ap;
  memcpy(ap, r.seq_state.data(), sizeof(SMState));
  lane_case_state<SeqPar>(a, *reinterpret_cast<SMState*>(ap));
  memcpy(r.seq_state.data(), ap, sizeof(SMState));
}

}
```

csrc/engine/lane_check.hip:

```cpp
#include <hip/hip_runtime.h>

#include <algorithm>

#include "engine.h"
#include "wave_par.h"
#include "sm_split.h"
#include "lane_check.h"

namespace asim {

template <class T, int N>
struct LaneReg<WavePar, T, N> {
  WarpReg<T> r;
  __device__ __forceinline__ explicit LaneReg(T (&arr)[N]) { r.load(arr); }
  __device__ __forceinline__ typename WarpReg<T>::Ref operator[](int w) { return r[w]; }
  __device__ __forceinline__ void store(T (&arr)[N]) { r.store(arr); }
};

__global__ __launch_bounds__(64) void lane_check_kernel(LaneArgs a, uint8_t* hbm_scratch, int scratch_hbm, SMState* st0,
                                                        SMState* st1, int split) {
  __shared__ __attribute__((aligned(16))) uint8_t lds[kLaneScratch];
  for (int i = (int)threadIdx.x; i < kLaneScratch; i += 64) lds[i] = kLaneCanary;
  __syncthreads();
  a.scratch = scratch_hbm ? hbm_scratch : lds;
  if (!st0) {
    lane_case_prim<WavePar>(a);
  } else if (split) {
    SmSplit sp(*st0, *st1);
    lane_case_state<WavePar>(a, sp);
  } else {
    lane_case_state<WavePar>(a, *st0);
  }
}

namespace {
void hip_ok(hipError_t e, const char* what) {
  if (e != hipSuccess) throw std::runtime_error(std::string("lane_policy_check: ") + what + ": " + hipGetErrorString(e));
}
struct DevBuf {
  void* p = nullptr;
  explicit DevBuf(size_t bytes) { hip_ok(hipMalloc(&p, bytes ? bytes : 16), "hipMalloc"); }
  ~DevBuf() {
    if (p) (void)hipFree(p);
  }
  DevBuf(const DevBuf&) = delete;
  DevBuf& operator=(const DevBuf&) = delete;
};
}

LaneCheckResult lane_policy_check(const std::string& name, int n, const std::vector<uint64_t>& val,
                                  const std::vector<uint64_t>& m) {
  const LanePlan p = lane_plan(name, n, val, m);
  LaneCheckResult r;
  lane_check_host(p, n, val, m, r);
  int ndev = 0;
  if (hipGetDeviceCount(&ndev) != hipSuccess || ndev <= 0) {
    (void)hipGetLastError();
    return r;
  }
  DevBuf d_val(val.size() * 8), d_m(m.size() * 8), d_out(p.nout * 8), d_scr(kLaneScratch);
  if (!val.empty()) hip_ok(hipMemcpy(d_val.p, val.data(), val.size() * 8, hipMemcpyHostToDevice), "copy values");
  if (!m.empty()) hip_ok(hipMemcpy(d_m.p, m.data(), m.size() * 8, hipMemcpyHostToDevice), "copy mask");
  hip_ok(hipMemset(d_out.p, 0, p.nout ? p.nout * 8 : 16), "clear outputs");
  hip_ok(hipMemset(d_scr.p, kLaneCanary, kLaneScratch), "fill scratch");
  std::unique_ptr<DevBuf> st0, st1;
  std::vector<uint64_t> img;
  if (p.state) {
    img.assign(sizeof(SMState) / 8, 0);
    lane_fill_pattern(img, lane_state_seed(p, val));
    st0.reset(new DevBuf(sizeof(SMState)));
    hip_ok(hipMemcpy(st0->p, img.data(), sizeof(SMState), hipMemcpyHostToDevice), "copy state");
    if (p.split) {
      st1.reset(new DevBuf(sizeof(SMState)));
      hip_ok(hipMemcpy(st1->p, img.data(), sizeof(SMState), hipMemcpyHostToDevice), "copy state");
    }
  }
  LaneArgs a{p.id, p.sub, n, (const uint64_t*)d_val.p, (int)val.size(), (const uint64_t*)d_m.p, (int)m.size(),
             (uint64_t*)d_out.p, nullptr};
  hipLaunchKernelGGL(lane_check_kernel, dim3(1), dim3(64), 0, 0, a, (uint8_t*)d_scr.p, p.scratch_hbm ? 1 : 0,
                     st0 ? (SMState*)st0->p : nullptr, st1 ? (SMState*)st1->p : nullptr, p.split ? 1 : 0);
  hip_ok(hipGetLastError(), "launch");
  hip_ok(hipDeviceSynchronize(), "kernel");
  r.wave.assign(p.nout, 0);
  if (p.nout) hip_ok(hipMemcpy(r.wave.data(), d_out.p, p.nout * 8, hipMemcpyDeviceToHost), "copy outputs");
  if (p.state) {
    std::vector<uint64_t> h0(img.size()), h1;
    hip_ok(hipMemcpy(h0.data(), st0->p, sizeof(SMState), hipMemcpyDeviceToHost), "copy state back");
    r.wave_state = h0;
    if (p.split) {
      h1.resize(img.size());
      hip_ok(hipMemcpy(h1.data(), st1->p, sizeof(SMState), hipMemcpyDeviceToHost), "copy state tail back");
      const size_t hot = kSmHotBytes / 8;
      std::copy(h1.begin() + hot, h1.end(), r.wave_state.begin() + hot);
      r.stray = !std::equal(h0.begin() + hot, h0.end(), img.begin() + hot) ||
                !std::equal(h1.begin(), h1.begin() + hot, img.begin());
    }
  }
  r.ran = true;
  return r;
}

}
```

csrc/engine/wave_par.h:

```cpp
#pragma once
#include <hip/hip_runtime.h>

#include "../model/hd.h"
#include "sm_view.h"

namespace asim {

struct WavePar {
  static constexpr int kLanes = 64;
  static __device__ __forceinline__ int lane() { return (int)(threadIdx.x & 63); }

  template <class F>
  static __device__ __forceinline__ uint64_t ballot(int n, F&& f) {
    const int l = lane();
    bool p = false;
    if (l < n) p = f(l);
    return (uint64_t)__ballot(p);
  }
  template <class F>
  static __device__ __forceinline__ void lane_loop(int n, F&& f) {
    for (int i = lane(); i < n; i += 64) f(i);
  }
  static __device__ __forceinline__ uint32_t red_sum(uint32_t v) {
    return wave_reduce(v, [](uint32_t a, uint32_t b) { return a + b; });
// ... 107 lines not shown
  template <int Ctrl>
  static __device__ __forceinline__ uint32_t dpp(uint32_t v) {
    return (uint32_t)__builtin_amdgcn_update_dpp((int)v, (int)v, Ctrl, 0xf, 0xf, false);
  }
  static __device__ __forceinline__ uint32_t rdl(uint32_t v, int l) {
    return (uint32_t)__builtin_amdgcn_readlane((int)v, l);
  }
  template <class Op>
  static __device__ __forceinline__ uint32_t row_reduce(uint32_t v, Op op) {
    v = op(v, dpp<0xB1>(v));
    v = op(v, dpp<0x4E>(v));
    v = op(v, dpp<0x141>(v));
    v = op(v, dpp<0x140>(v));
    return v;
  }
  template <class Op>
  static __device__ __forceinline__ uint32_t wave_reduce(uint32_t v, Op op) {
    v = row_reduce(v, op);
    return op(op(rdl(v, 0), rdl(v, 16)), op(rdl(v, 32), rdl(v, 48)));
  }
  static __device__ __forceinline__ bool kless(uint32_t ah, uint32_t al, uint32_t ai, uint32_t bh, uint32_t bl,
                                               uint32_t bi) {
    return ah < bh || (ah == bh && (al < bl || (al == bl && ai < bi)));
  }
  template <int Ctrl>
  static __device__ __forceinline__ void kstep(uint32_t& h, uint32_t& l, uint32_t& i) {
    const uint32_t oh = dpp<Ctrl>(h), ol = dpp<Ctrl>(l), oi = dpp<Ctrl>(i);
    if (kless(oh, ol, oi, h, l, i)) {
      h = oh;
      l = ol;
      i = oi;
    }
  }
  template <class F>
  static __device__ __forceinline__ int argmin(int n, F&& key) {
    uint64_t best = ~0ull;
    uint32_t bi = 0x7fffffffu;
    for (int i = lane(); i < n; i += 64) {
      uint64_t k = key(i);
      if (k != ~0ull && (k < best || (k == best && (uint32_t)i < bi))) {
        best = k;
        bi = (uint32_t)i;
      }
    }
    uint32_t h = (uint32_t)(best >> 32), l = (uint32_t)best;
    kstep<0xB1>(h, l, bi);
    kstep<0x4E>(h, l, bi);
    kstep<0x141>(h, l, bi);
    kstep<0x140>(h, l, bi);
    uint32_t rh = rdl(h, 0), rl = rdl(l, 0), ri = rdl(bi, 0);
#pragma unroll
    for (int r = 16; r < 64; r += 16) {
      const uint32_t oh = rdl(h, r), ol = rdl(l, r), oi = rdl(bi, r);
      if (kless(oh, ol, oi, rh, rl, ri)) {
        rh = oh;
        rl = ol;
        ri = oi;
      }
    }
    return (rh == ~0u && rl == ~0u) ? -1 : (int)ri;
  }
  template <class T>
  struct LaneVal {
    T v;
    __device__ __forceinline__ T self(int) const { return v; }
    __device__ __forceinline__ T at(int i) const {
      static_assert(sizeof(T) % 4 == 0, "LaneVal: word-multiple types");
      uint32_t w[sizeof(T) / 4];
      __builtin_memcpy(w, &v, sizeof(T));
#pragma unroll
      for (int k = 0; k < (int)(sizeof(T) / 4); ++k) w[k] = rdl(w[k], i);
      T r;
      __builtin_memcpy(&r, w, sizeof(T));
      return r;
    }
  };
  template <class T, class F>
  static __device__ __forceinline__ LaneVal<T> lanes(int n, F&& f) {
    LaneVal<T> r;
    if (lane() < n) r.v = f(lane());
    else __builtin_memset(&r.v, 0, sizeof(T));
    return r;
  }
  template <class F>
  static __device__ __forceinline__ uint64_t order16(int n, uint32_t mask, F&& key) {
    const int l = lane();
    const bool mine = l < n && (mask >> l & 1u);
    const uint32_t k = mine ? (uint32_t)key(l) : 0u;
    uint32_t r = 0;
    for (uint32_t m = mask; m;) {
      const int j = __builtin_ctz(m);
      m &= m - 1;
      const uint32_t kj = rdl(k, j);
      r += (j != l && (kj < k || (kj == k && j < l))) ? 1u : 0u;
    }
    const uint64_t v = mine ? ((uint64_t)(uint32_t)l << (4 * r)) : 0ull;
    auto o = [](uint32_t a, uint32_t b) { return a | b; };
    const uint32_t lo = wave_reduce((uint32_t)v, o), hi = wave_reduce((uint32_t)(v >> 32), o);
    return ((uint64_t)hi << 32) | lo;
  }
  template <class F>
  static __device__ __forceinline__ int find_first(int n, F&& pred) {
    const int l = lane();
    for (int b = 0; b < n; b += 256) {
      bool p0 = false, p1 = false, p2 = false, p3 = false;
      if (b + l < n) p0 = pred(b + l);
      if (b + 64 < n && b + 64 + l < n) p1 = pred(b + 64 + l);
      if (b + 128 < n && b + 128 + l < n) p2 = pred(b + 128 + l);
      if (b + 192 < n && b + 192 + l < n) p3 = pred(b + 192 + l);
      const uint64_t m0 = (uint64_t)__ballot(p0), m1 = (uint64_t)__ballot(p1), m2 = (uint64_t)__ballot(p2),
                     m3 = (uint64_t)__ballot(p3);
      if (m0) return b + __builtin_ctzll(m0);
      if (m1) return b + 64 + __builtin_ctzll(m1);
      if (m2) return b + 128 + __builtin_ctzll(m2);
      if (m3) return b + 192 + __builtin_ctzll(m3);
    }
    return -1;
  }
  template <class F>
  static __device__ __forceinline__ uint32_t sum(int n, F&& f) {
    uint32_t s = 0;
    for (int i = lane(); i < n; i += 64) s += f(i);
    return wave_reduce(s, [](uint32_t a, uint32_t b) { return a + b; });
  }
  template <class F>
  static __device__ __forceinline__ uint32_t vmax(int n, F&& f) {
    uint32_t s = 0;
    for (int i = lane(); i < n; i += 64) {
      uint32_t v = f(i);
      s = v > s ? v : s;
    }
    return wave_reduce(s, [](uint32_t a, uint32_t b) { return a > b ? a : b; });
  }
  template <class F>
  static __device__ __forceinline__ uint64_t vor(int n, F&& f) {
    uint64_t s = 0;
    for (int i = lane(); i < n; i += 64) s |= f(i);
    auto o = [](uint32_t a, uint32_t b) { return a | b; };
    const uint32_t lo = wave_reduce((uint32_t)s, o), hi = wave_reduce((uint32_t)(s >> 32), o);
    return ((uint64_t)hi << 32) | lo;
  }
  static __device__ __forceinline__ void min32(uint32_t* p, uint32_t v) {
    (void)__hip_atomic_fetch_min(p, v, __ATOMIC_RELAXED, __HIP_MEMORY_SCOPE_WORKGROUP);
  }
  static __device__ __forceinline__ void add64(uint64_t* p, uint64_t v) {
    if (lane() == 0) (void)__hip_atomic_fetch_add(p, v, __ATOMIC_RELAXED, __HIP_MEMORY_SCOPE_AGENT);
  }
  template <class F, class G>
  static __device__ __forceinline__ uint32_t scan(int n, F&& val, G&& out) {
    uint32_t carry = 0;
    const int l = lane();
    for (int b = 0; b < n; b += 64) {
      const int i = b + l;
      uint32_t v = i < n ? val(i) : 0u;
      uint32_t inc = v;
      inc += (uint32_t)__builtin_amdgcn_update_dpp(0, (int)inc, 0x111, 0xf, 0xf, false);
      inc += (uint32_t)__builtin_amdgcn_update_dpp(0, (int)inc, 0x112, 0xf, 0xf, false);
      inc += (uint32_t)__builtin_amdgcn_update_dpp(0, (int)inc, 0x114, 0xf, 0xf, false);
      inc += (uint32_t)__builtin_amdgcn_update_dpp(0, (int)inc, 0x118, 0xf, 0xf, false);
      const uint32_t t0 = rdl(inc, 15), t1 = rdl(inc, 31), t2 = rdl(inc, 47), t3 = rdl(inc, 63);
      const int row = l >> 4;
      inc += row == 0 ? 0u : row == 1 ? t0 : row == 2 ? t0 + t1 : t0 + t1 + t2;
      if (i < n) out(i, carry + inc - v);
      carry += t0 + t1 + t2 + t3;
    }
    return carry;
// ... 5 lines not shown
```

csrc/model/hd.h:

```cpp
#pragma once
#include <stdint.h>

#if defined(__HIP__)
#include <hip/hip_runtime.h>
#define SIM_HD __host__ __device__
#define SIM_HDI __host__ __device__ __forceinline__
#define SIM_HDN __host__ __device__ inline __attribute__((noinline))
#else
#define SIM_HDN inline
#define SIM_HD
#define SIM_HDI inline
#endif

namespace asim {

SIM_HDI int popc64(uint64_t x) { return __builtin_popcountll(x); }
SIM_HDI int ffs64(uint64_t x) { return x ? __builtin_ctzll(x) : -1; }
SIM_HDI uint64_t rotr64(uint64_t x, unsigned r, unsigned n) {
  if (r == 0) return x;
  uint64_t m = (n == 64) ? ~0ull : ((1ull << n) - 1);
  x &= m;
  return ((x >> r) | (x << (n - r))) & m;
}
template <class T>
// ... 14 lines not shown
  static SIM_HDI void lane_loop(int n, F&& f) {
    for (int i = 0; i < n; ++i) f(i);
  }
  static SIM_HDI uint32_t red_sum(uint32_t v) { return v; }
  static SIM_HDI uint32_t red_or(uint32_t v) { return v; }
  static SIM_HDI uint64_t red_sum64(uint64_t v) { return v; }
  static SIM_HDI uint64_t red_min64(uint64_t v) { return v; }
  static SIM_HDI uint64_t red_max64(uint64_t v) { return v; }
  template <class F>
  static SIM_HDI uint64_t ballot_m(uint64_t mask, F&& f) {
    uint64_t m = 0;
    for (uint64_t r = mask; r; r &= r - 1) {
      const int i = __builtin_ctzll(r);
      if (f(i)) m |= 1ull << i;
    }
    return m;
  }
  template <class F>
  static SIM_HDI void each_m(uint64_t mask, F&& f) {
    for (uint64_t r = mask; r; r &= r - 1) f(__builtin_ctzll(r));
  }
  template <class F>
  static SIM_HDI void each(int n, F&& f) {
    for (int i = 0; i < n; ++i) f(i);
  }
  template <class F>
  static SIM_HDI void one(F&& f) { f(); }
  template <class T>
  static SIM_HDI void fetch_copy(T* dst, const T* src, int n) {
    for (int i = 0; i < n; ++i) dst[i] = src[i];
  }
  static SIM_HDI void fetch_wait() {}
  static SIM_HDI void sync() {}
  static SIM_HDI void prof(int) {}
  static SIM_HDI void tick(int) {}
  template <class T>
  static SIM_HDI T uni(T v) { return v; }
  template <class S, class F>
  static SIM_HDI void view(S& s, F&& f) { f(s); }
  template <class F>
  static SIM_HDI int argmin(int n, F&& key) {
    uint64_t best = ~0ull;
    int bi = -1;
    for (int i = 0; i < n; ++i) {
      uint64_t k = key(i);
      if (k != ~0ull && (bi < 0 || k < best)) {
        best = k;
        bi = i;
      }
    }
    return bi;
  }
  template <class F>
  static SIM_HDI int find_first(int n, F&& pred) {
    for (int i = 0; i < n; ++i)
      if (pred(i)) return i;
    return -1;
  }
  template <class F>
  static SIM_HDI uint32_t sum(int n, F&& f) {
    uint32_t s = 0;
    for (int i = 0; i < n; ++i) s += f(i);
    return s;
  }
  template <class F>
  static SIM_HDI uint32_t vmax(int n, F&& f) {
    uint32_t s = 0;
    for (int i = 0; i < n; ++i) {
      uint32_t v = f(i);
      s = v > s ? v : s;
    }
    return s;
  }
  template <class T, class F>
  struct Lanes {
    F f;
    SIM_HDI T self(int i) const { return f(i); }
    SIM_HDI T at(int i) const { return f(i); }
  };
  template <class T, class F>
  static SIM_HDI Lanes<T, F> lanes(int, F f) {
    return Lanes<T, F>{f};
  }
  template <class F, class G>
  static SIM_HDI uint32_t scan(int n, F&& val, G&& out) {
    uint32_t acc = 0;
    for (int i = 0; i < n; ++i) {
      uint32_t v = val(i);
      out(i, acc);
      acc += v;
    }
    return acc;
  }
  template <class F>
  static SIM_HDI uint64_t vor(int n, F&& f) {
    uint64_t s = 0;
    for (int i = 0; i < n; ++i) s |= f(i);
    return s;
  }
  static SIM_HDI void min32(uint32_t* p, uint32_t v) {
    if (v < *p) *p = v;
  }
  static SIM_HDI void add64(uint64_t* p, uint64_t v) { *p += v; }
  template <class F>
  static SIM_HDI uint64_t order16(int n, uint32_t mask, F&& key) {
    uint64_t ord = 0;
    for (int i = 0; i < n; ++i) {
      if (!(mask >> i & 1u)) continue;
      const uint32_t ki = key(i);
      uint32_t r = 0;
      for (int j = 0; j < n; ++j)
        if ((mask >> j & 1u) && j != i) {
          const uint32_t kj = key(j);
          r += (kj < ki || (kj == ki && j < i)) ? 1u : 0u;
        }
      ord |= (uint64_t)i << (4 * r);
    }
    return ord;
  }
};

}
```

csrc/model/sm.h:

```cpp
#pragma once
#include <stddef.h>
#if !defined(__HIP_DEVICE_COMPILE__)
#include <stdexcept>
#include <stdio.h>
#endif

#include "addrdec.h"

namespace asim {



enum WarpFlags : uint8_t {
  WF_ACTIVE = 1,
  WF_EXITING = 2,
  WF_BARRIER = 4,
  WF_MEMBAR = 8,
  WF_WAITCNT = 16,
  WF_IMISS = 32,
};

struct HitEnt {
  uint8_t warp;
  uint8_t slot;
// ... 205 lines not shown
  WbEnt wb[kWbRing][kWbSlot];
  uint8_t hit_cnt[kHitRing];
  HitEnt hit[kHitRing][kHitSlot];
  L1Line l1[kMaxL1Lines];
  L1Mshr mshr[kMaxL1Mshr];
  L1Pend pend[kMaxPend];
  L1Line il1[kMaxIL1Lines];
  L1Mshr imshr[kMaxIL1Mshr];
  L1Line cl1[kMaxCL1Lines];
  L1Mshr cmshr[kMaxCL1Mshr];
  SIM_HDI void sadd(uint32_t k, uint64_t d) { reinterpret_cast<uint64_t*>(&st)[k] += d; }
  SIM_HDI uint64_t sget(uint32_t k) const { return reinterpret_cast<const uint64_t*>(&st)[k]; }
  SIM_HDI void sset(uint32_t k, uint64_t v) { reinterpret_cast<uint64_t*>(&st)[k] = v; }
  template <uint32_t LO, uint32_t HI>
  SIM_HDI void sadd_r(uint32_t k, uint64_t d) { sadd(k, d); }
};
#define SK(f) ((uint32_t)(offsetof(::asim::SMStats, f) / 8))
#define SADD_IN(s, f, n, i, d) (s).template sadd_r<SK(f), SK(f) + (n)>(SK(f) + (uint32_t)(i), (d))
constexpr int kStatWords = (int)(sizeof(SMStats) / 8);
static_assert(kStatWords <= 256, "SM statistics: up to four 64-lane register words on the GPU engine");
template <class S>
SIM_HDI uint64_t* s_scratch_key(S& s) { return s.skey; }
template <class S>
SIM_HDI uint32_t* s_scratch_ref(S& s) { return s.sref; }
template <class S>
SIM_HDI uint32_t* s_scratch_rank(S& s) { return s.srank; }

struct SmCtx {
  const SimCfg* cfg;
  const KernelTab* kt;
  Pkt* outbox;
  uint32_t* outcnt;
  uint32_t out_cap;
  uint32_t n_src_sm;
  const uint64_t* rt_st = nullptr;
};

SIM_HDI uint32_t wb_width(const SimCfg& c) { return c.ex_wb_width < (uint32_t)kWbSlot ? c.ex_wb_width : (uint32_t)kWbSlot; }

SIM_HDI bool sb_test(const uint64_t* sb, uint8_t r) { return r && ((sb[r >> 6] >> (r & 63)) & 1ull); }
SIM_HDI void sb_set(uint64_t* sb, uint8_t r) {
  if (r) sb[r >> 6] |= 1ull << (r & 63);
}
SIM_HDI void sb_clr(uint64_t* sb, uint8_t r) {
  if (r) sb[r >> 6] &= ~(1ull << (r & 63));
}
template <size_t N>
SIM_HDI bool sbt(const uint64_t (&sb)[N][4], uint32_t w, uint8_t r) { return sb_test(sb[w], r); }
template <size_t N>
SIM_HDI void sbs(uint64_t (&sb)[N][4], uint32_t w, uint8_t r) { sb_set(sb[w], r); }
template <size_t N>
SIM_HDI void sbc(uint64_t (&sb)[N][4], uint32_t w, uint8_t r) { sb_clr(sb[w], r); }
template <size_t N>
SIM_HDI void sbz(uint64_t (&sb)[N][4], uint32_t w) { sb[w][0] = sb[w][1] = sb[w][2] = sb[w][3] = 0; }

template <class P, class S>
SIM_HDI void sm_reset(S& s, uint32_t id) {
  s.id = id;
}

template <class S>
SIM_HDI CacheGeom l1_geom(const SimCfg& c, const S& s) {
  CacheGeom g = c.l1;
  const uint32_t sets = s.l1_sets;
  if (sets) {
    g.nsets = sets;
    g.assoc = s.l1_assoc;
  }
  return g;
}

template <class S>
SIM_HDI bool sm_can_send(const S& s, const SimCfg& c) {
  return s.outq_n < c.icnt_in_pkts && s.outstanding + s.outq_n < c.icnt_out_limit;
}
template <class S>
SIM_HDI bool sm_can_send_n(const S& s, const SimCfg& c, uint32_t n) {
  return s.outq_n + n <= c.icnt_in_pkts && s.outstanding + s.outq_n + n <= c.icnt_out_limit;
}
constexpr uint32_t kTagL1Writeback = 0x20000000u;
template <class S>
SIM_HDI void sm_send(S& s, const SimCfg& c, uint8_t type, uint64_t line, uint8_t sectors,
                     uint16_t bytes, uint32_t tag) {
  AddrTlx t = addr_decode(c, line);
  Pkt& p = s.outq[(s.outq_head + s.outq_n) % kOutQ];
  p.addr = line;
  p.t = 0;
  p.tag = tag;
  p.src = (uint16_t)s.id;
  p.dst = (uint16_t)l2_slice_of(c, s.id, t.sub);
  p.type = type;
  p.sectors = sectors;
  p.size = (type == P_WR) ? (uint16_t)(8 + bytes) : (uint16_t)8;
  p.aux = 0;
  s.outq_n++;
}

template <class S>
SIM_HDI uint32_t wr_packets(const SimCfg& c, uint8_t sectors) {
  if (c.l1_wr_req_bytes != 64) return 1u;
  return ((sectors & 3u) && (sectors & 12u)) ? 2u : 1u;
}
template <class S>
SIM_HDI uint32_t sm_send_write(S& s, const SimCfg& c, uint64_t line, uint8_t sectors, uint16_t bytes, uint32_t tag) {
  if (wr_packets<S>(c, sectors) == 1) {
    sm_send(s, c, P_WR, line, sectors, bytes, tag);
    return 1;
  }
  const uint8_t lo = sectors & 3u, hi = sectors & 12u;
  const uint32_t n = (uint32_t)popc64(sectors);
  const uint16_t blo = (uint16_t)((uint32_t)bytes * (uint32_t)popc64(lo) / n);
  sm_send(s, c, P_WR, line, lo, blo, tag);
  sm_send(s, c, P_WR, line, hi, (uint16_t)(bytes - blo), tag);
  return 2;
}

SIM_HDI bool rt_inj_ok(const SimCfg& c, uint64_t t0_fs, int64_t allow0, uint64_t used, uint32_t nfl, uint64_t now_fs) {
  const uint64_t k = now_fs > t0_fs ? fdiv(now_fs - t0_fs, c.dv_icnt) : 0;
  return (int64_t)(used + nfl) <= allow0 + (int64_t)(k < (1ull << 40) ? k : (1ull << 40));
}

template <class P, class S>
SIM_HDI void sm_inject(S& s, const SmCtx& x, uint64_t now) {
  const SimCfg& c = *x.cfg;
  if (P::uni(s.outq_n) == 0) return;
  if (now < P::uni(s.out_port_free)) return;
  Pkt p = P::uni(s.outq[P::uni(s.outq_head)]);
  uint32_t nflits = (p.size + c.flit_size - 1) / c.flit_size;
  uint64_t done = now + nflits - 1;
  uint32_t dst = p.dst;
  uint32_t slot = dst * x.n_src_sm + s.id;
  uint32_t n = P::uni(s.ocnt[dst]);
  if (n >= x.out_cap) return;
  const uint32_t cpc = c.cores_per_cluster ? c.cores_per_cluster : 1;
  if (c.link_contention == 2 &&
      !rt_inj_ok(c, P::uni(s.inj_t0_fs), P::uni(s.inj_allow0), P::uni(s.inj_used), nflits * cpc, core_fs(c, now))) {
    s.sadd(SK(icnt_inj_stall), 1);
    return;
  }
  if (c.link_contention == 2) s.inj_used = s.inj_used + (uint64_t)nflits * cpc;
  s.ocnt[dst] = n + 1;
  p.t = core_fs(c, done) + icnt_pkt_lat_fs(c, s.id, dst);
  s.min_emit = amin(s.min_emit, p.t);
  if (trace_sm_on(c, TS_INTERCONNECT, s.id)) P::one([&] { trace_put(c, s.id, now, EV_PKT_SEND, (uint16_t)dst, p.addr); });
  P::one([&] {
    x.outbox[(uint64_t)slot * x.out_cap + n] = p;
    x.outcnt[slot] = n + 1;
  });
  s.outq_head = (s.outq_head + 1) % kOutQ;
  s.outq_n--;
  s.out_port_free = now + nflits;
  s.outstanding++;
  s.sadd(SK(pkts_out), 1);
  s.sadd(SK(bytes_out), p.size);
}

template <class P, class S>
SIM_HDI void sm_writeback(S& s, const SimCfg& c, uint64_t now) {
  uint32_t slot = (uint32_t)(now % kWbRing);
  if (!((P::uni((uint64_t)s.wb_occ[slot >> 6]) >> (slot & 63)) & 1ull)) return;
  uint32_t n = P::uni(s.wb_cnt[slot]);
  for (uint32_t i = 0; i < n; ++i) {
    WbEnt e = P::uni(s.wb[slot][i]);
    if (trace_sm_on(c, TS_SCOREBOARD, s.id))
      P::one([&] {
        if (e.dst0) trace_put(c, s.id, now, EV_SB_RELEASE, e.warp, e.dst0 - 1u);
        if (e.dst1) trace_put(c, s.id, now, EV_SB_RELEASE, e.warp, e.dst1 - 1u);
      });
    sbc(s.w_sb, e.warp, e.dst0);
    sbc(s.w_sb, e.warp, e.dst1);
    s.w_inflight[e.warp]--;
    s.sadd(SK(rf_writes), (e.dst0 != 0) + (e.dst1 != 0));
  }
  if (n) s.last_progress = now;
  s.wb_cnt[slot] = 0;
  s.wb_occ[slot >> 6] &= ~(1ull << (slot & 63));
}

template <class S>
SIM_HDI void sm_load_slot_done(S& s, uint32_t w, uint32_t slot, uint64_t now) {
  sbc(s.w_sb, w, s.w_slot_dst[w][slot][0]);
  sbc(s.w_sb, w, s.w_slot_dst[w][slot][1]);
  s.sadd(SK(rf_writes), (s.w_slot_dst[w][slot][0] != 0) + (s.w_slot_dst[w][slot][1] != 0));
  s.w_slot_used[w] &= (uint8_t)~(1u << slot);
  s.w_slot_lds[w] &= (uint8_t)~(1u << slot);
  s.w_loads[w]--;
  s.w_inflight[w]--;
  s.last_progress = now;
}

template <class S>
SIM_HDI bool waitcnt_met(S& s, uint32_t w) {
  const uint32_t wt = s.w_wait[w];
  const uint32_t lds_ld = (uint32_t)__builtin_popcount((uint32_t)s.w_slot_lds[w]);
  const uint32_t vm = (uint32_t)s.w_loads[w] - lds_ld + (uint32_t)s.w_stores[w];
  const uint32_t lgkm = lds_ld + (uint32_t)s.w_lds_st[w];
  return vm <= (wt & 0xffu) && lgkm <= (wt >> 8);
}

template <class P, class S>
SIM_HDI void sm_hit_complete(S& s, uint64_t now) {
  uint32_t slot = (uint32_t)(now % kHitRing);
  if (!((P::uni((uint64_t)s.hit_occ[slot >> 6]) >> (slot & 63)) & 1ull)) return;
  uint32_t n = P::uni(s.hit_cnt[slot]);
  for (uint32_t i = 0; i < n; ++i) {
    HitEnt e = P::uni(s.hit[slot][i]);
    if (e.kind == 0) {
      if (--s.w_slot_pend[e.warp][e.slot] == 0) sm_load_slot_done(s, e.warp, e.slot, now);
    } else {
      s.w_inflight[e.warp]--;
      s.w_lds_st[e.warp]--;
      s.last_progress = now;
    }
  }
  s.hit_cnt[slot] = 0;
  s.hit_occ[slot >> 6] &= ~(1ull << (slot & 63));
}

template <class S>
SIM_HDI bool hit_push(S& s, uint64_t when, uint8_t warp, uint8_t slot, uint8_t kind) {
  uint32_t r = (uint32_t)(when % kHitRing);
  if (s.hit_cnt[r] >= kHitSlot) return false;
  s.hit_occ[r >> 6] |= 1ull << (r & 63);
  HitEnt& e = s.hit[r][s.hit_cnt[r]++];
  e.warp = warp;
  e.slot = slot;
  e.kind = kind;
  e.pad = 0;
  return true;
}

// ... 539 lines not shown
          ++got;
          ++grants;
        }
      }
      if (got) {
        nr -= got;
        b = (b & ~(0xffull << 40)) | ((uint64_t)nr << 40);
        s.oc_banks[i] = b;
        s.sadd(SK(rf_reads), got);
        if (nr == 0) rmask &= ~(1u << i);
      }
      if (nr) s.sadd(SK(oc_bank_conflicts), nr);
    }
    s.oc_read_mask = rmask;
  }
}

template <class P, class S>
SIM_HDI void sm_dispatch(S& s, const SmCtx& x, uint64_t now) {
  const SimCfg& c = *x.cfg;
  const KernelTab* x_kt = x.kt;
  const int noc = (int)amin<uint32_t>(c.oc_units, kMaxOC);
  const uint32_t wbw = wb_width(c);
  const uint32_t ready = P::uni(s.oc_mask & ~s.oc_read_mask);
  if (!ready) return;
  const int n = popc64(ready);
  const uint64_t ord =
      n == 1 ? (uint64_t)ffs64(ready) : P::order16(noc, ready, [&](int i) -> uint32_t { return s.oc_age[i]; });
  for (int r = 0; r < n; ++r) {
    const int best = (int)((ord >> (4 * r)) & 15u);
    const uint64_t info = P::uni((uint64_t)s.oc_info[best]);
    const uint32_t u = (uint32_t)(info >> 16) & 0xffu;
    if (u == U_MEM) {
      if (P::uni(s.ldst.busy)) continue;
      const TInst li = P::uni(s.oc_inst[best]);
      s.ldst.inst = li;
      s.ldst.busy = 1;
      s.ldst.warp = (uint8_t)(info & 0xffu);
      if (li.space != S_SHARED && li.width && li.mem != kNoMem) {
        const KernelDesc& kacc = x_kt->k[P::uni((uint32_t)s.w_end[info & 0xffu]) >> kSlotShift];
        const TAcc* accs = kacc.accs;
        P::fetch_copy(&s.ldst_acc[0], &accs[li.mem & kacc.amask], (int)amin<uint32_t>(li.width, kMaxAccess));
      }
      s.ldst.slot = (uint8_t)((info >> 24) & 0xffu);
      s.ldst.next = 0;
      s.ldst.start = (uint32_t)now;
      if (c.l1_addr_lanes && li.space != S_SHARED && li.space != S_CONST && li.width) {
        const uint32_t pf = P::uni(s.ldst.port_free);
        const uint32_t from = (int32_t)(pf - (uint32_t)now) > 0 ? pf : (uint32_t)now;
        s.ldst.port_free = from + ((uint32_t)popc64(li.mask) + c.l1_addr_lanes - 1) / c.l1_addr_lanes;
      }
      s.sadd(SK(mem_insn), 1);
      s.oc_mask &= ~(1u << best);
      continue;
    }
    const uint32_t sched = (uint32_t)(info >> 8) & 0xffu;
    const uint32_t cnt = c.unit_count[u] ? c.unit_count[u] : 1;
    uint32_t phys = sched < cnt ? sched : sched % cnt;
    if (phys >= (uint32_t)kMaxSched) phys %= kMaxSched;
    const uint32_t fi = u * (uint32_t)kMaxSched + phys;
    const uint32_t nf = P::uni((uint32_t)s.fu_next[fi]);
    if ((int32_t)(nf - (uint32_t)now) > 0) continue;
    uint32_t lat = (uint32_t)(info >> 32) & 0xffffu;
    if (!lat) lat = 1;
    if (lat >= (uint32_t)kWbRing) lat = kWbRing - 1;
    const uint32_t slot = (uint32_t)((now + lat) % kWbRing);
    const uint32_t nwb = P::uni(s.wb_cnt[slot]);
    if (nwb >= wbw) { s.sadd(SK(pipe_stall), 1); continue; }
    s.wb_cnt[slot] = (uint8_t)(nwb + 1);
    const uint64_t bk = P::uni((uint64_t)s.oc_banks[best]);
    WbEnt& e = s.wb[slot][nwb];
    s.wb_occ[slot >> 6] |= 1ull << (slot & 63);
    e.warp = (uint8_t)(info & 0xffu);
    e.dst0 = (uint8_t)(bk >> 48);
    e.dst1 = (uint8_t)(bk >> 56);
    e.pad = 0;
    const uint32_t ii = (uint32_t)(info >> 48) & 0xffu;
    s.fu_next[fi] = (uint32_t)now + (ii ? ii : 1);
    s.oc_mask &= ~(1u << best);
  }
}

template <class P, class S>
SIM_HDI void sm_alloc_collectors(S& s, const SimCfg& c) {
  const int noc = (int)amin<uint32_t>(c.oc_units, kMaxOC);
  const uint32_t nsched = c.n_sched;
  const uint32_t per = (c.sub_core && nsched) ? (noc / nsched ? noc / nsched : 1) : (uint32_t)noc;
  uint64_t pend = P::uni(s.idoc_mask);
  uint32_t ocm = P::uni(s.oc_mask);
  while (pend) {
    const int bit = ffs64(pend);
    pend &= pend - 1;
    const uint32_t sc = (uint32_t)bit / U_COUNT, u = (uint32_t)bit % U_COUNT;
    uint32_t lo = c.sub_core ? (sc * per) % noc : 0;
    uint32_t hi = c.sub_core ? lo + per : (uint32_t)noc;
    if (hi > (uint32_t)noc) hi = noc;
    const uint32_t grp = ((hi >= 32 ? 0xffffffffu : ((1u << hi) - 1)) & ~((1u << lo) - 1));
    const uint32_t freem = grp & ~ocm;
    if (!freem) continue;
    const int f = ffs64(freem);
    ocm |= 1u << f;
    s.oc_mask = ocm;
    const uint64_t meta = P::uni((uint64_t)s.idoc_meta[bit]);
    const TInst rin = P::uni(s.idoc_inst[bit]);
    const uint32_t rw = (uint32_t)(meta & 0xffu);
    s.oc_inst[f] = rin;
    uint64_t bk = 0;
    uint32_t nread = 0;
    for (int j = 0; j < 5; ++j) {
      const uint8_t reg = rin.src[j];
      const uint32_t bank = reg ? reg_bank(c, sc, rw, reg - 1u) : 0xffu;
      bk |= (uint64_t)(bank & 0xffu) << (8 * j);
      nread += reg ? 1u : 0u;
    }
    bk |= (uint64_t)nread << 40 | (uint64_t)rin.dst[0] << 48 | (uint64_t)rin.dst[1] << 56;
    s.oc_banks[f] = bk;
    s.oc_info[f] = (uint64_t)rw | (uint64_t)sc << 8 | (uint64_t)u << 16 | ((meta >> 8) & 0xffull) << 24 |
                   (uint64_t)rin.lat << 32 | (uint64_t)rin.ii << 48;
    s.oc_age[f] = (uint32_t)(meta >> 32);
    if (nread) s.oc_read_mask |= 1u << f;
    s.idoc_mask &= ~(1ull << bit);
  }
}

template <class P, class S>
SIM_HDI void sm_barrier_check(S& s, uint32_t cta) {
  uint32_t live = s.cta_live[cta] - s.cta_nexit[cta];
  if (s.cta_bar[cta] > 0 && s.cta_bar[cta] >= live) {
    const uint32_t base = s.cta_wbase[cta], nw = s.cta_nw[cta];
    for (uint32_t w = base; w < base + nw && w < (uint32_t)kMaxWarps; ++w)
      s.w_flags[w] &= (uint8_t)~WF_BARRIER;
    s.cta_bar[cta] = 0;
  }
}

SIM_HDI uint32_t mod_small(uint32_t x, uint32_t n) {
  if (x < n) return x;
  x -= n;
  return x < n ? x : x % n;
}
SIM_HDI uint32_t sched_of(uint32_t w, uint32_t nsched) {
  return (nsched & (nsched - 1)) == 0 ? (w & (nsched - 1)) : w % nsched;
}

template <class S>
SIM_HDI bool warp_sb_ok(const S& s, int w, const TInst& in) {
  for (int j = 0; j < 5; ++j)
    if (sbt(s.w_sb, w, in.src[j])) return false;
  return !sbt(s.w_sb, w, in.dst[0]) && !sbt(s.w_sb, w, in.dst[1]);
}
template <class S>
SIM_HDI bool warp_can_issue_nosb(const S& s, const SimCfg& c, int w, const TInst& in, uint32_t nsched,
                                 uint64_t idoc_busy) {
  uint8_t f = s.w_flags[w];
  if (!(f & WF_ACTIVE) || (f & (WF_EXITING | WF_BARRIER | WF_MEMBAR | WF_WAITCNT))) return false;
  if (s.w_ibuf[w] == 0) return false;
  uint32_t u = unit_of(c, in.cls);
  uint32_t sc = sched_of((uint32_t)w, nsched);
  if (in.cls == OC_EXIT || in.cls == OC_BARRIER || in.cls == OC_MEMBAR || in.cls == OC_NOP || (in.flags & F_WAITCNT))
    return true;
  if (idoc_busy >> (sc * U_COUNT + u) & 1ull) return false;
  if (u == U_MEM && in.cls == OC_LOAD && s.w_slot_used[w] == 0xff) return false;
  return true;
}
template <class S>
SIM_HDI bool warp_can_issue_i(const S& s, const SimCfg& c, int w, const TInst& in, uint32_t nsched,
                              uint64_t idoc_busy) {
  return warp_can_issue_nosb(s, c, w, in, nsched, idoc_busy) && warp_sb_ok(s, w, in);
}
template <class S>
SIM_HDI bool warp_can_issue(const S& s, const SimCfg& c, const KernelTab& kt, int w, uint32_t nsched,
                            uint64_t idoc_busy) {
  if (!(s.w_flags[w] & WF_ACTIVE) || s.w_ibuf[w] == 0) return false;
  const TInst in = s.w_win[w][s.w_head[w] & (kWin - 1)];
  return warp_can_issue_i(s, c, w, in, nsched, idoc_busy);
}

template <class S>
SIM_HDI bool warp_issue_due(const S& s, const SimCfg& c, int w, uint64_t now) {
  return c.warp_issue_interval <= 1 || now >= s.w_issue_ok[w];
}

template <class P, class S>
SIM_HDI int sm_issue_one(S& s, const SmCtx& x, uint64_t now, uint32_t sc, uint32_t w, const TInst& in,
                         uint32_t hidx) {
  const SimCfg& c = *x.cfg;
  if (trace_sm_on(c, TS_WARP_SCHEDULER, s.id))
    P::one([&] { trace_put(c, s.id, now, EV_ISSUE, (uint16_t)w, (uint64_t)in.pc | (uint64_t)in.opcode << 32); });
  s.w_head[w] = hidx + 1;
  s.w_ibuf[w] = (uint8_t)(P::uni((uint8_t)s.w_ibuf[w]) - 1);
  s.sadd(SK(warp_insn), 1);
  s.sadd(SK(thread_insn), (uint64_t)popc64(in.mask));
  SADD_IN(s, cls_insn, OC_COUNT, in.cls < OC_COUNT ? in.cls : OC_ALU, 1);
  SADD_IN(s, sq_insn, 8, sq_class(in), 1);
  if (in.space == S_CONST) s.sadd(SK(power_acc) + PWR_CONST_OPERAND, 1);
  {
    const uint32_t pk = (uint32_t)(in.flags >> 4);
    if (pk) SADD_IN(s, power_acc, 16, pk, pk == PWR_SALU ? 1ull : (uint64_t)popc64(in.mask));
  }
  s.last_progress = now;
  const uint32_t cta = P::uni((uint8_t)s.w_cta[w]);
  if (in.cls == OC_EXIT) {
    if (hidx + 1 >= P::uni((uint32_t)s.w_end[w])) {
      s.w_flags[w] |= WF_EXITING;
      s.cta_nexit[cta]++;
// ... 672 lines not shown
```

Before: 300,900.

## Specialize kernels on link contention, parallelize collector allocation, defer packet routing

The engine kernel gets a compile-time kLinks template flag, so builds without link contention drop the link-pass branches and link state pointers. Batching is disabled when links are on. Operand-collector allocation is rewritten to assign free collectors across wavefront lanes with ballots and a new gather primitive instead of a serial loop, with the old version kept as a reference for lane checks. Packet destination decoding moves from enqueue to send time. Together these aim to reduce per-cycle SM overhead, at the cost of more kernel instantiations and a riskier parallel allocation order.

```diff
diff --git a/build_native.py b/build_native.py
--- a/build_native.py
+++ b/build_native.py
@@ -30,7 +30,8 @@
     "csrc/parallel/linksim.cc",
 ]
 HIP_SRC = ["csrc/engine/gpu_engine.hip", "csrc/engine/engine_k_lds.hip", "csrc/engine/engine_k_prof.hip",
-           "csrc/engine/engine_k_global.hip", "csrc/engine/engine_k_split.hip", "csrc/engine/engine_k_split2.hip", "csrc/engine/ingest_mfma.hip",
+           "csrc/engine/engine_k_global.hip", "csrc/engine/engine_k_split.hip", "csrc/engine/engine_k_split2.hip",
+           "csrc/engine/engine_k_links.hip", "csrc/engine/engine_k_links_prof.hip", "csrc/engine/ingest_mfma.hip",
            "csrc/engine/lane_check.hip", "csrc/engine/icnt_sweep.hip"]
 STUB_SRC = ["csrc/engine/gpu_stub.cc"]
 
diff --git a/csrc/bindings/py_asim.cc b/csrc/bindings/py_asim.cc
--- a/csrc/bindings/py_asim.cc
+++ b/csrc/bindings/py_asim.cc
@@ -639,6 +639,7 @@
             return py::bytes(reinterpret_cast<const char*>(v.data()), v.size() * 8);
           };
           if (!r.seq_state.empty()) d["seq_state"] = bytes_of(r.seq_state);
+          if (!r.ref_state.empty()) d["ref_state"] = bytes_of(r.ref_state);
           if (r.ran) {
             d["wave"] = r.wave;
             d["stray"] = r.stray;
diff --git a/csrc/engine/engine.h b/csrc/engine/engine.h
--- a/csrc/engine/engine.h
+++ b/csrc/engine/engine.h
@@ -167,6 +167,7 @@
 struct LaneCheckResult {
   std::vector<uint64_t> seq, wave;
   std::vector<uint64_t> seq_state, wave_state;
+  std::vector<uint64_t> ref_state;
   bool ran = false;
   bool stray = false;
   uint32_t stat_words = (uint32_t)kStatWords;
diff --git a/csrc/engine/engine_k_global.hip b/csrc/engine/engine_k_global.hip
--- a/csrc/engine/engine_k_global.hip
+++ b/csrc/engine/engine_k_global.hip
@@ -2,13 +2,13 @@
 
 namespace asim {
 
-template __global__ void engine_kernel<WavePar, true, kModeGlobal>(GpuArgs);
+template __global__ void engine_kernel<WavePar, true, kModeGlobal, false>(GpuArgs);
 
 __global__ void ASIM_ENGINE_KERNEL_ATTRS engine_batch_kernel(const GpuArgs* __restrict__ jobs,
                                                              const uint16_t* __restrict__ block_job) {
   const uint32_t j = block_job[blockIdx.x];
   const GpuArgs a = jobs[j];
-  engine_body<WavePar, true, kModeGlobal>(a, blockIdx.x - a.block0);
+  engine_body<WavePar, true, kModeGlobal, false>(a, blockIdx.x - a.block0);
 }
 
 ASIM_ENGINE_CFG_UPLOAD(global)
diff --git a/csrc/engine/engine_k_lds.hip b/csrc/engine/engine_k_lds.hip
--- a/csrc/engine/engine_k_lds.hip
+++ b/csrc/engine/engine_k_lds.hip
@@ -2,8 +2,8 @@
 
 namespace asim {
 
-template __global__ void engine_kernel<WavePar, false, kModeLds>(GpuArgs);
-template __global__ void engine_kernel<WavePar, true, kModeLds>(GpuArgs);
+template __global__ void engine_kernel<WavePar, false, kModeLds, false>(GpuArgs);
+template __global__ void engine_kernel<WavePar, true, kModeLds, false>(GpuArgs);
 
 ASIM_ENGINE_CFG_UPLOAD(lds)
 
diff --git a/csrc/engine/engine_k_links.hip b/csrc/engine/engine_k_links.hip
--- /dev/null
+++ b/csrc/engine/engine_k_links.hip
@@ -0,0 +1,16 @@
+#include "engine_kernel.h"
+
+namespace asim {
+
+template __global__ void engine_kernel<WavePar, false, kModeLds, true>(GpuArgs);
+template __global__ void engine_kernel<WavePar, true, kModeLds, true>(GpuArgs);
+template __global__ void engine_kernel<WavePar, true, kModeGlobal, true>(GpuArgs);
+template __global__ void engine_kernel<WavePar, true, kModeSplit, true>(GpuArgs);
+
+__global__ void ASIM_SPLIT2_KERNEL_ATTRS engine_split2_links_kernel(GpuArgs a) {
+  engine_body<WavePar, true, kModeSplit, true>(a, blockIdx.x);
+}
+
+ASIM_ENGINE_CFG_UPLOAD(links)
+
+}
diff --git a/csrc/engine/engine_k_links_prof.hip b/csrc/engine/engine_k_links_prof.hip
--- /dev/null
+++ b/csrc/engine/engine_k_links_prof.hip
@@ -0,0 +1,12 @@
+#include "engine_kernel.h"
+
+namespace asim {
+
+template __global__ void engine_kernel<WaveParProf, false, kModeLds, true>(GpuArgs);
+template __global__ void engine_kernel<WaveParProf, true, kModeLds, true>(GpuArgs);
+template __global__ void engine_kernel<WaveParProf, true, kModeGlobal, true>(GpuArgs);
+template __global__ void engine_kernel<WaveParProf, true, kModeSplit, true>(GpuArgs);
+
+ASIM_ENGINE_CFG_UPLOAD(links_prof)
+
+}
diff --git a/csrc/engine/engine_k_prof.hip b/csrc/engine/engine_k_prof.hip
--- a/csrc/engine/engine_k_prof.hip
+++ b/csrc/engine/engine_k_prof.hip
@@ -2,10 +2,10 @@
 
 namespace asim {
 
-template __global__ void engine_kernel<WaveParProf, false, kModeLds>(GpuArgs);
-template __global__ void engine_kernel<WaveParProf, true, kModeLds>(GpuArgs);
-template __global__ void engine_kernel<WaveParProf, true, kModeGlobal>(GpuArgs);
-template __global__ void engine_kernel<WaveParProf, true, kModeSplit>(GpuArgs);
+template __global__ void engine_kernel<WaveParProf, false, kModeLds, false>(GpuArgs);
+template __global__ void engine_kernel<WaveParProf, true, kModeLds, false>(GpuArgs);
+template __global__ void engine_kernel<WaveParProf, true, kModeGlobal, false>(GpuArgs);
+template __global__ void engine_kernel<WaveParProf, true, kModeSplit, false>(GpuArgs);
 
 ASIM_ENGINE_CFG_UPLOAD(prof)
 
diff --git a/csrc/engine/engine_k_split.hip b/csrc/engine/engine_k_split.hip
--- a/csrc/engine/engine_k_split.hip
+++ b/csrc/engine/engine_k_split.hip
@@ -2,13 +2,13 @@
 
 namespace asim {
 
-template __global__ void engine_kernel<WavePar, true, kModeSplit>(GpuArgs);
+template __global__ void engine_kernel<WavePar, true, kModeSplit, false>(GpuArgs);
 
 __global__ void ASIM_ENGINE_KERNEL_ATTRS engine_batch_split_kernel(const GpuArgs* __restrict__ jobs,
                                                                    const uint16_t* __restrict__ block_job) {
   const uint32_t j = block_job[blockIdx.x];
   const GpuArgs a = jobs[j];
-  engine_body<WavePar, true, kModeSplit>(a, blockIdx.x - a.block0);
+  engine_body<WavePar, true, kModeSplit, false>(a, blockIdx.x - a.block0);
 }
 
 ASIM_ENGINE_CFG_UPLOAD(split)
diff --git a/csrc/engine/engine_k_split2.hip b/csrc/engine/engine_k_split2.hip
--- a/csrc/engine/engine_k_split2.hip
+++ b/csrc/engine/engine_k_split2.hip
@@ -2,10 +2,8 @@
 
 namespace asim {
 
-#define ASIM_SPLIT2_KERNEL_ATTRS __launch_bounds__(64) __attribute__((amdgpu_waves_per_eu(2, 2)))
-
 __global__ void ASIM_SPLIT2_KERNEL_ATTRS engine_split2_kernel(GpuArgs a) {
-  engine_body<WavePar, true, kModeSplit>(a, blockIdx.x);
+  engine_body<WavePar, true, kModeSplit, false>(a, blockIdx.x);
 }
 
 ASIM_ENGINE_CFG_UPLOAD(split2)
diff --git a/csrc/engine/engine_kernel.h b/csrc/engine/engine_kernel.h
--- a/csrc/engine/engine_kernel.h
+++ b/csrc/engine/engine_kernel.h
@@ -215,7 +215,7 @@
   __syncthreads();
 }
 
-template <class P, bool kSliced, int kMode>
+template <class P, bool kSliced, int kMode, bool kLinks>
 __device__ __forceinline__ void engine_body(const GpuArgs& a, const uint32_t b) {
   constexpr bool kGlobal = kMode == kModeGlobal, kSplit = kMode == kModeSplit;
   const SimCfg& c = g_cfg[a.cfg_slot];
@@ -295,14 +295,14 @@
   sx.kt = &kt;
   sx.out_cap = a.cap_req;
   sx.n_src_sm = c.n_sm;
-  sx.rt_st = c.link_contention == 2 ? a.link_free : nullptr;
+  sx.rt_st = kLinks && c.link_contention == 2 ? a.link_free : nullptr;
   MemCtx mx;
   mx.cfg = &c;
   mx.out_cap = a.cap_rep;
   mx.n_src_sub = c.n_subpart;
   mx.ovf = a.ovf;
   mx.ovf_cap = a.ovf_cap;
-  mx.rt_st = c.link_contention == 2 ? a.link_free : nullptr;
+  mx.rt_st = kLinks && c.link_contention == 2 ? a.link_free : nullptr;
   mx.mall = nullptr;
   uint64_t epoch = a.epoch0, cycle = a.cycle0;
   uint64_t t_work0 = a.ework ? __builtin_amdgcn_s_memtime() : 0;
@@ -352,7 +352,7 @@
     }
     uint32_t was_last = 0;
     if (!grid_barrier_b(a.ctl, b, a.nblocks, nbar++, &was_last)) break;
-    if (a.link_free) {
+    if (kLinks && a.link_free) {
       const bool rt_par = c.link_contention == 2 && c.router_pass == 1;
       if (rt_par) {
         if (b < 2) {
@@ -444,9 +444,9 @@
 
 #define ASIM_ENGINE_KERNEL_ATTRS __launch_bounds__(64) __attribute__((amdgpu_waves_per_eu(1, 1)))
 
-template <class P, bool kSliced, int kMode>
+template <class P, bool kSliced, int kMode, bool kLinks>
 __global__ void ASIM_ENGINE_KERNEL_ATTRS engine_kernel(GpuArgs a) {
-  engine_body<P, kSliced, kMode>(a, blockIdx.x);
+  engine_body<P, kSliced, kMode, kLinks>(a, blockIdx.x);
 }
 
 __global__ void ASIM_ENGINE_KERNEL_ATTRS engine_batch_kernel(const GpuArgs* __restrict__ jobs,
@@ -455,6 +455,8 @@
                                                                    const uint16_t* __restrict__ block_job);
 
 __global__ void engine_split2_kernel(GpuArgs a);
+__global__ void engine_split2_links_kernel(GpuArgs a);
+#define ASIM_SPLIT2_KERNEL_ATTRS __launch_bounds__(64) __attribute__((amdgpu_waves_per_eu(2, 2)))
 
 #define ASIM_ENGINE_CFG_UPLOAD(name)                                                         \
   hipError_t engine_upload_cfg_##name(const SimCfg& c, int slot) {                          \
diff --git a/csrc/engine/gpu_engine.hip b/csrc/engine/gpu_engine.hip
--- a/csrc/engine/gpu_engine.hip
+++ b/csrc/engine/gpu_engine.hip
@@ -32,19 +32,22 @@
       throw std::runtime_error(std::string("HIP error: ") + hipGetErrorString(e_) + " at " #x);    \
   } while (0)
 
-extern template __global__ void engine_kernel<WavePar, false, kModeLds>(GpuArgs);
-extern template __global__ void engine_kernel<WavePar, true, kModeLds>(GpuArgs);
-extern template __global__ void engine_kernel<WaveParProf, false, kModeLds>(GpuArgs);
-extern template __global__ void engine_kernel<WaveParProf, true, kModeLds>(GpuArgs);
-extern template __global__ void engine_kernel<WavePar, true, kModeGlobal>(GpuArgs);
-extern template __global__ void engine_kernel<WaveParProf, true, kModeGlobal>(GpuArgs);
-extern template __global__ void engine_kernel<WavePar, true, kModeSplit>(GpuArgs);
-extern template __global__ void engine_kernel<WaveParProf, true, kModeSplit>(GpuArgs);
+#define ASIM_ENGINE_BUILDS(X) \
+  X(WavePar, false, kModeLds) X(WavePar, true, kModeLds) X(WaveParProf, false, kModeLds) X(WaveParProf, true, kModeLds) \
+  X(WavePar, true, kModeGlobal) X(WaveParProf, true, kModeGlobal) X(WavePar, true, kModeSplit) X(WaveParProf, true, kModeSplit)
+#define ASIM_ENGINE_EXTERN(P, sliced, mode)                                            \
+  extern template __global__ void engine_kernel<P, sliced, mode, false>(GpuArgs); \
+  extern template __global__ void engine_kernel<P, sliced, mode, true>(GpuArgs);
+ASIM_ENGINE_BUILDS(ASIM_ENGINE_EXTERN)
+#undef ASIM_ENGINE_EXTERN
+#undef ASIM_ENGINE_BUILDS
 hipError_t engine_upload_cfg_lds(const SimCfg& c, int slot);
 hipError_t engine_upload_cfg_prof(const SimCfg& c, int slot);
 hipError_t engine_upload_cfg_global(const SimCfg& c, int slot);
 hipError_t engine_upload_cfg_split(const SimCfg& c, int slot);
 hipError_t engine_upload_cfg_split2(const SimCfg& c, int slot);
+hipError_t engine_upload_cfg_links(const SimCfg& c, int slot);
+hipError_t engine_upload_cfg_links_prof(const SimCfg& c, int slot);
 
 namespace {
 
@@ -141,7 +144,7 @@
     int occ = 0;
     const void* f = mode == kModeGlobal ? (const void*)engine_batch_kernel
                     : split_waves() == 2 ? (const void*)engine_split2_kernel
-                                         : (const void*)engine_kernel<WavePar, true, kModeSplit>;
+                                         : (const void*)engine_kernel<WavePar, true, kModeSplit, false>;
     const size_t lds = mode == kModeGlobal ? kLdsBytesGlobal : kLdsBytesSplit;
     if (hipOccupancyMaxActiveBlocksPerMultiprocessor(&occ, f, 64, (int)lds) != hipSuccess) occ = 2;
     g_occ_api = occ;
@@ -587,8 +590,10 @@
     global_ = mode_ == kModeGlobal;
     lds_ = global_ ? kLdsBytesGlobal : mode_ == kModeSplit ? kLdsBytesSplit : kLdsBytes;
     sliced_ = nblocks_ < c.n_sm + c.n_mem;
-    for (const void* f : {(const void*)engine_kernel<WavePar, false, kModeLds>, (const void*)engine_kernel<WaveParProf, false, kModeLds>,
-                          (const void*)engine_kernel<WavePar, true, kModeLds>, (const void*)engine_kernel<WaveParProf, true, kModeLds>})
+    for (const void* f : {(const void*)engine_kernel<WavePar, false, kModeLds, false>, (const void*)engine_kernel<WaveParProf, false, kModeLds, false>,
+                          (const void*)engine_kernel<WavePar, true, kModeLds, false>, (const void*)engine_kernel<WaveParProf, true, kModeLds, false>,
+                          (const void*)engine_kernel<WavePar, false, kModeLds, true>, (const void*)engine_kernel<WaveParProf, false, kModeLds, true>,
+                          (const void*)engine_kernel<WavePar, true, kModeLds, true>, (const void*)engine_kernel<WaveParProf, true, kModeLds, true>})
       HIPCHECK(hipFuncSetAttribute(f, hipFuncAttributeMaxDynamicSharedMemorySize, (int)kLdsBytes));
     slots_ = engine_block_slots(mode_);
     batch_ = (global_ || mode_ == kModeSplit) && !profiling_env() && gpu_batch_on();
@@ -646,6 +651,7 @@
                               icnt_scratch_words(c, cap_req_, cap_rep_) > kMaxIcntScratchWords))
       throw std::runtime_error("-icnt_link_contention: topology or mailboxes too large for the link pass");
     n_links_ = icnt_contention_on(c) ? (size_t)icnt_state_words(c, cap_req_, cap_rep_) : 0;
+    if (n_links_) batch_ = false;
     if (n_links_) {
       pool_alloc(&d_links_, sizeof(uint64_t) * (n_links_ + kIcntStatWords));
       HIPCHECK(hipMemset(d_links_, 0, sizeof(uint64_t) * (n_links_ + kIcntStatWords)));
@@ -740,36 +746,9 @@
         HIPCHECK(sub.err);
       } else {
       CuPool::get().acquire((int)(nblocks_ * slots_));
-      hipError_t le;
-      if (mode_ == kModeSplit && profiling_) {
-        variant_ = "split_prof";
-        hipLaunchKernelGGL((engine_kernel<WaveParProf, true, kModeSplit>), dim3(nblocks_), dim3(64), lds_, stream_, a);
-      } else if (mode_ == kModeSplit && split_waves() == 2) {
-        variant_ = "split2";
-        hipLaunchKernelGGL(engine_split2_kernel, dim3(nblocks_), dim3(64), lds_, stream_, a);
-      } else if (mode_ == kModeSplit) {
-        variant_ = "split";
-        hipLaunchKernelGGL((engine_kernel<WavePar, true, kModeSplit>), dim3(nblocks_), dim3(64), lds_, stream_, a);
-      } else if (global_ && profiling_) {
-        variant_ = "global_prof";
-        hipLaunchKernelGGL((engine_kernel<WaveParProf, true, kModeGlobal>), dim3(nblocks_), dim3(64), lds_, stream_, a);
-      } else if (global_) {
-        variant_ = "global";
-        hipLaunchKernelGGL((engine_kernel<WavePar, true, kModeGlobal>), dim3(nblocks_), dim3(64), lds_, stream_, a);
-      } else if (profiling_ && sliced_) {
-        variant_ = "lds_sliced_prof";
-        hipLaunchKernelGGL((engine_kernel<WaveParProf, true, kModeLds>), dim3(nblocks_), dim3(64), lds_, stream_, a);
-      } else if (profiling_) {
-        variant_ = "lds_prof";
-        hipLaunchKernelGGL((engine_kernel<WaveParProf, false, kModeLds>), dim3(nblocks_), dim3(64), lds_, stream_, a);
-      } else if (sliced_) {
-        variant_ = "lds_sliced";
-        hipLaunchKernelGGL((engine_kernel<WavePar, true, kModeLds>), dim3(nblocks_), dim3(64), lds_, stream_, a);
-      } else {
-        variant_ = "lds";
-        hipLaunchKernelGGL((engine_kernel<WavePar, false, kModeLds>), dim3(nblocks_), dim3(64), lds_, stream_, a);
-      }
-      le = hipGetLastError();
+      if (a.link_free) launch_build<true>(a);
+      else launch_build<false>(a);
+      const hipError_t le = hipGetLastError();
       ++launches_;
       hipError_t ce = hipMemcpyAsync(h_ctl_, d_ctl_, sizeof(GpuCtl), hipMemcpyDeviceToHost, stream_);
       hipError_t se = hipEventRecord(done_ev_, stream_);
@@ -1054,6 +1033,37 @@
   }
 
  private:
+  template <bool kLinks>
+  void launch_build(const GpuArgs& a) {
+    if (mode_ == kModeSplit && profiling_) {
+      variant_ = "split_prof";
+      hipLaunchKernelGGL((engine_kernel<WaveParProf, true, kModeSplit, kLinks>), dim3(nblocks_), dim3(64), lds_, stream_, a);
+    } else if (mode_ == kModeSplit && split_waves() == 2) {
+      variant_ = "split2";
+      hipLaunchKernelGGL(kLinks ? engine_split2_links_kernel : engine_split2_kernel, dim3(nblocks_), dim3(64), lds_, stream_, a);
+    } else if (mode_ == kModeSplit) {
+      variant_ = "split";
+      hipLaunchKernelGGL((engine_kernel<WavePar, true, kModeSplit, kLinks>), dim3(nblocks_), dim3(64), lds_, stream_, a);
+    } else if (global_ && profiling_) {
+      variant_ = "global_prof";
+      hipLaunchKernelGGL((engine_kernel<WaveParProf, true, kModeGlobal, kLinks>), dim3(nblocks_), dim3(64), lds_, stream_, a);
+    } else if (global_) {
+      variant_ = "global";
+      hipLaunchKernelGGL((engine_kernel<WavePar, true, kModeGlobal, kLinks>), dim3(nblocks_), dim3(64), lds_, stream_, a);
+    } else if (profiling_ && sliced_) {
+      variant_ = "lds_sliced_prof";
+      hipLaunchKernelGGL((engine_kernel<WaveParProf, true, kModeLds, kLinks>), dim3(nblocks_), dim3(64), lds_, stream_, a);
+    } else if (profiling_) {
+      variant_ = "lds_prof";
+      hipLaunchKernelGGL((engine_kernel<WaveParProf, false, kModeLds, kLinks>), dim3(nblocks_), dim3(64), lds_, stream_, a);
+    } else if (sliced_) {
+      variant_ = "lds_sliced";
+      hipLaunchKernelGGL((engine_kernel<WavePar, true, kModeLds, kLinks>), dim3(nblocks_), dim3(64), lds_, stream_, a);
+    } else {
+      variant_ = "lds";
+      hipLaunchKernelGGL((engine_kernel<WavePar, false, kModeLds, kLinks>), dim3(nblocks_), dim3(64), lds_, stream_, a);
+    }
+  }
   void upload_cfg() {
     HIPCHECK(hipMemcpy(d_cfg_, &c_, sizeof(SimCfg), hipMemcpyHostToDevice));
     HIPCHECK(engine_upload_cfg_lds(c_, cfg_slot_));
@@ -1061,6 +1071,8 @@
     HIPCHECK(engine_upload_cfg_global(c_, cfg_slot_));
     HIPCHECK(engine_upload_cfg_split(c_, cfg_slot_));
     HIPCHECK(engine_upload_cfg_split2(c_, cfg_slot_));
+    HIPCHECK(engine_upload_cfg_links(c_, cfg_slot_));
+    HIPCHECK(engine_upload_cfg_links_prof(c_, cfg_slot_));
   }
   void release() {
     auto fr = [](void* p) {
@@ -1279,9 +1291,9 @@
     int mode;
     const void* f;
     size_t lds;
-  } ms[] = {{"lds", kModeLds, (const void*)engine_kernel<WavePar, false, kModeLds>, kLdsBytes},
+  } ms[] = {{"lds", kModeLds, (const void*)engine_kernel<WavePar, false, kModeLds, false>, kLdsBytes},
             {"global", kModeGlobal, (const void*)engine_batch_kernel, kLdsBytesGlobal},
-            {"split", kModeSplit, (const void*)engine_kernel<WavePar, true, kModeSplit>, kLdsBytesSplit},
+            {"split", kModeSplit, (const void*)engine_kernel<WavePar, true, kModeSplit, false>, kLdsBytesSplit},
             {"split2", kModeSplit, (const void*)engine_split2_kernel, kLdsBytesSplit}};
   for (const auto& m : ms) {
     auto& o = out[m.name];
@@ -1335,7 +1347,7 @@
 EngineKernelInfo gpu_engine_kernel_info() {
   EngineKernelInfo k;
   hipFuncAttributes fa;
-  if (hipFuncGetAttributes(&fa, (const void*)engine_kernel<WavePar, false, kModeLds>) != hipSuccess) return k;
+  if (hipFuncGetAttributes(&fa, (const void*)engine_kernel<WavePar, false, kModeLds, false>) != hipSuccess) return k;
   k.num_regs = fa.numRegs;
   k.local_bytes = (int)fa.localSizeBytes;
   k.shared_static = (int)fa.sharedSizeBytes;
diff --git a/csrc/engine/lane_check.h b/csrc/engine/lane_check.h
--- a/csrc/engine/lane_check.h
+++ b/csrc/engine/lane_check.h
@@ -14,7 +14,7 @@
 enum LaneCase : int {
   LC_BALLOT = 0, LC_BALLOT_M, LC_EACH_M, LC_RED_SUM, LC_RED_OR, LC_SUM, LC_VMAX, LC_VOR, LC_RED_SUM64, LC_RED_MIN64,
   LC_RED_MAX64, LC_ARGMIN, LC_FIND_FIRST, LC_SCAN, LC_ORDER16, LC_LANES, LC_UNI, LC_FETCH, LC_REG, LC_SB, LC_STAT,
-  LC_VIEW, LC_MIN32
+  LC_VIEW, LC_MIN32, LC_OC_ALLOC
 };
 
 constexpr int kLaneScratch = 1024;
@@ -29,6 +29,7 @@
   int nm;
   uint64_t* out;
   uint8_t* scratch;
+  const SimCfg* cfg = nullptr;
 };
 
 struct LanePlan {
@@ -407,8 +408,31 @@
 }
 
 template <class P, class S>
+SIM_HD void lane_oc_alloc_prep(const LaneArgs& a, S& s) {
+  const SimCfg& c = *a.cfg;
+  const uint32_t noc = amin<uint32_t>(c.oc_units, kMaxOC), fill = (uint32_t)a.val[5];
+  const uint64_t few = a.val[6];
+  P::one([&] {
+    uint64_t valid = 0;
+    for (uint32_t sc = 0; sc < c.n_sched; ++sc) valid |= ((1ull << U_COUNT) - 1) << (sc * U_COUNT);
+    const uint32_t all = (1u << noc) - 1u;
+    s.idoc_mask = fill == 2 ? valid : fill == 4 ? (s.idoc_mask & valid & few) : (s.idoc_mask & valid);
+    s.oc_mask = fill == 1 ? all : fill == 3 ? 0u : (s.oc_mask & all);
+    s.oc_read_mask = s.oc_read_mask & s.oc_mask;
+  });
+  P::sync();
+}
+template <class P, class S>
+SIM_HD void lane_oc_alloc_case(const LaneArgs& a, S& s) {
+  lane_oc_alloc_prep<P>(a, s);
+  const SimCfg& c = *a.cfg;
+  P::view(s, [&](auto& v) { sm_alloc_collectors<P>(v, c); });
+}
+
+template <class P, class S>
 SIM_HD void lane_case_state(const LaneArgs& a, S& s) {
-  if (a.id == LC_SB) lane_sb_case<P>(a, s);
+  if (a.id == LC_OC_ALLOC) lane_oc_alloc_case<P>(a, s);
+  else if (a.id == LC_SB) lane_sb_case<P>(a, s);
   else if (a.id == LC_STAT) lane_stat_case<P>(a, s);
   else lane_view_case<P>(a, s);
 }
@@ -510,6 +534,20 @@
         }
     bad("unknown register type / extent");
   }
+  if (name == "oc_alloc") {
+    p.state = true;
+    p.id = LC_OC_ALLOC;
+    need(n == 0 || n == 1, "n: 0 = SMState, 1 = SmSplit");
+    p.split = n == 1;
+    need(nv >= 7, "seed, n_sched, oc_units, sub_core, reg_banks, fill, mask");
+    need(val[1] >= 1 && val[1] <= (uint64_t)kMaxSched, "1 <= n_sched <= 4");
+    need(val[2] >= 1 && val[2] <= (uint64_t)kMaxOC, "1 <= oc_units <= 16");
+    need(val[3] <= 1, "sub_core 0 / 1");
+    need(val[4] >= 1 && val[4] <= 64, "1 <= reg_banks <= 64");
+    need(val[5] <= 4, "fill 0..4");
+    p.nout = 0;
+    return p;
+  }
   if (name == "sb" || name == "stat" || name == "view") {
     p.state = true;
     need(n == 0 || n == 1, "n: 0 = SMState, 1 = SmSplit");
@@ -542,6 +580,17 @@
   return p;
 }
 
+inline SimCfg lane_cfg(const LanePlan& p, const std::vector<uint64_t>& val) {
+  SimCfg c{};
+  if (p.id == LC_OC_ALLOC) {
+    c.n_sched = (uint32_t)val[1];
+    c.oc_units = (uint32_t)val[2];
+    c.sub_core = (uint32_t)val[3];
+    c.reg_banks = (uint32_t)val[4];
+  }
+  return c;
+}
+
 inline uint64_t lane_state_seed(const LanePlan& p, const std::vector<uint64_t>& val) {
   return val[p.id == LC_SB ? 192 : 0];
 }
@@ -556,6 +605,8 @@
   if (reinterpret_cast<uintptr_t>(v) % 16) ++v;
   if (!val.empty()) memcpy(v, val.data(), val.size() * 8);
   LaneArgs a{p.id, p.sub, n, v, (int)val.size(), m.data(), (int)m.size(), r.seq.data(), scratch};
+  const SimCfg cfg = lane_cfg(p, val);
+  a.cfg = &cfg;
   if (!p.state) {
     lane_case_prim<SeqPar>(a);
     return;
@@ -568,6 +619,16 @@
   uint64_t* ap = al.data();
   if (reinterpret_cast<uintptr_t>(ap) % 16) ++ap;
   memcpy(ap, r.seq_state.data(), sizeof(SMState));
+  if (p.id == LC_OC_ALLOC) {
+    std::vector<uint64_t> bl(words + 2);
+    uint64_t* bp = bl.data();
+    if (reinterpret_cast<uintptr_t>(bp) % 16) ++bp;
+    memcpy(bp, r.seq_state.data(), sizeof(SMState));
+    SMState& ref = *reinterpret_cast<SMState*>(bp);
+    lane_oc_alloc_prep<SeqPar>(a, ref);
+    sm_alloc_collectors_seq<SeqPar>(ref, cfg);
+    r.ref_state.assign(bp, bp + words);
+  }
   lane_case_state<SeqPar>(a, *reinterpret_cast<SMState*>(ap));
   memcpy(r.seq_state.data(), ap, sizeof(SMState));
 }
diff --git a/csrc/engine/lane_check.hip b/csrc/engine/lane_check.hip
--- a/csrc/engine/lane_check.hip
+++ b/csrc/engine/lane_check.hip
@@ -77,6 +77,10 @@
   }
   LaneArgs a{p.id, p.sub, n, (const uint64_t*)d_val.p, (int)val.size(), (const uint64_t*)d_m.p, (int)m.size(),
              (uint64_t*)d_out.p, nullptr};
+  const SimCfg cfg = lane_cfg(p, val);
+  DevBuf d_cfg(sizeof(SimCfg));
+  hip_ok(hipMemcpy(d_cfg.p, &cfg, sizeof(SimCfg), hipMemcpyHostToDevice), "copy configuration");
+  a.cfg = (const SimCfg*)d_cfg.p;
   hipLaunchKernelGGL(lane_check_kernel, dim3(1), dim3(64), 0, 0, a, (uint8_t*)d_scr.p, p.scratch_hbm ? 1 : 0,
                      st0 ? (SMState*)st0->p : nullptr, st1 ? (SMState*)st1->p : nullptr, p.split ? 1 : 0);
   hip_ok(hipGetLastError(), "launch");
diff --git a/csrc/engine/wave_par.h b/csrc/engine/wave_par.h
--- a/csrc/engine/wave_par.h
+++ b/csrc/engine/wave_par.h
@@ -213,6 +213,35 @@
     else __builtin_memset(&r.v, 0, sizeof(T));
     return r;
   }
+  template <class T, class R, class F>
+  static __device__ __forceinline__ LaneVal<T> gather(uint64_t mask, const WarpReg<R>& r, F&& idx) {
+    static_assert(sizeof(R) <= 8, "gather: register fields of at most 64 bits");
+    const int l = lane();
+    const uint32_t j = (mask >> l) & 1ull ? (uint32_t)idx(l) : 0u;
+    const uint64_t u = (uint64_t)r.v;
+    uint32_t lo = 0, hi = 0;
+    for (uint64_t m = mask; m; m &= m - 1) {
+      const int f = __builtin_ctzll(m);
+      const int src = (int)(rdl(j, f) & 63u);
+      const uint32_t a = rdl((uint32_t)u, src);
+      lo = l == f ? a : lo;
+      if constexpr (sizeof(R) == 8) {
+        const uint32_t b = rdl((uint32_t)(u >> 32), src);
+        hi = l == f ? b : hi;
+      }
+    }
+    LaneVal<T> out;
+    out.v = (T)(R)(((uint64_t)hi << 32) | lo);
+    return out;
+  }
+  template <class T, class A, class F>
+  static __device__ __forceinline__ LaneVal<T> gather(uint64_t mask, const A& arr, F&& idx) {
+    LaneVal<T> out;
+    const int l = lane();
+    if ((mask >> l) & 1ull) out.v = (T)arr[idx(l)];
+    else __builtin_memset(&out.v, 0, sizeof(T));
+    return out;
+  }
   template <class F>
   static __device__ __forceinline__ uint64_t order16(int n, uint32_t mask, F&& key) {
     const int l = lane();
diff --git a/csrc/model/hd.h b/csrc/model/hd.h
--- a/csrc/model/hd.h
+++ b/csrc/model/hd.h
@@ -120,6 +120,16 @@
   static SIM_HDI Lanes<T, F> lanes(int, F f) {
     return Lanes<T, F>{f};
   }
+  template <class T, class A, class F>
+  struct Gathered {
+    const A& a;
+    F idx;
+    SIM_HDI T self(int i) const { return (T)a[idx(i)]; }
+  };
+  template <class T, class A, class F>
+  static SIM_HDI Gathered<T, A, F> gather(uint64_t, const A& arr, F idx) {
+    return Gathered<T, A, F>{arr, idx};
+  }
   template <class F, class G>
   static SIM_HDI uint32_t scan(int n, F&& val, G&& out) {
     uint32_t acc = 0;
diff --git a/csrc/model/sm.h b/csrc/model/sm.h
--- a/csrc/model/sm.h
+++ b/csrc/model/sm.h
@@ -311,13 +311,12 @@
 template <class S>
 SIM_HDI void sm_send(S& s, const SimCfg& c, uint8_t type, uint64_t line, uint8_t sectors,
                      uint16_t bytes, uint32_t tag) {
-  AddrTlx t = addr_decode(c, line);
   Pkt& p = s.outq[(s.outq_head + s.outq_n) % kOutQ];
   p.addr = line;
   p.t = 0;
   p.tag = tag;
   p.src = (uint16_t)s.id;
-  p.dst = (uint16_t)l2_slice_of(c, s.id, t.sub);
+  p.dst = 0;
   p.type = type;
   p.sectors = sectors;
   p.size = (type == P_WR) ? (uint16_t)(8 + bytes) : (uint16_t)8;
@@ -354,10 +353,12 @@
   const SimCfg& c = *x.cfg;
   if (P::uni(s.outq_n) == 0) return;
   if (now < P::uni(s.out_port_free)) return;
-  Pkt p = P::uni(s.outq[P::uni(s.outq_head)]);
+  const uint32_t head = P::uni(s.outq_head);
+  Pkt p = P::uni(s.outq[head]);
   uint32_t nflits = (p.size + c.flit_size - 1) / c.flit_size;
   uint64_t done = now + nflits - 1;
-  uint32_t dst = p.dst;
+  p.dst = (uint16_t)l2_slice_of(c, s.id, addr_decode(c, p.addr).sub);
+  const uint32_t dst = p.dst;
   uint32_t slot = dst * x.n_src_sm + s.id;
   uint32_t n = P::uni(s.ocnt[dst]);
   if (n >= x.out_cap) return;
@@ -376,6 +377,7 @@
     x.outbox[(uint64_t)slot * x.out_cap + n] = p;
     x.outcnt[slot] = n + 1;
   });
+  s.outq[head].dst = (uint16_t)dst;
   s.outq_head = (s.outq_head + 1) % kOutQ;
   s.outq_n--;
   s.out_port_free = now + nflits;
@@ -1081,7 +1083,7 @@
 }
 
 template <class P, class S>
-SIM_HDI void sm_alloc_collectors(S& s, const SimCfg& c) {
+SIM_HDI void sm_alloc_collectors_seq(S& s, const SimCfg& c) {
   const int noc = (int)amin<uint32_t>(c.oc_units, kMaxOC);
   const uint32_t nsched = c.n_sched;
   const uint32_t per = (c.sub_core && nsched) ? (noc / nsched ? noc / nsched : 1) : (uint32_t)noc;
@@ -1120,6 +1122,72 @@
     if (nread) s.oc_read_mask |= 1u << f;
     s.idoc_mask &= ~(1ull << bit);
   }
+}
+
+
+template <class P, class S>
+SIM_HDI void sm_alloc_collectors(S& s, const SimCfg& c) {
+  const uint64_t pend = P::uni(s.idoc_mask);
+  if (!pend) return;
+  const uint32_t noc = amin<uint32_t>(c.oc_units, kMaxOC);
+  const uint32_t ocm = P::uni(s.oc_mask);
+  const uint32_t freem = ((1u << noc) - 1u) & ~ocm;
+  if (!freem) return;
+  const uint32_t nsched = amin<uint32_t>(c.n_sched, kMaxSched);
+  const bool sub = c.sub_core && nsched;
+  const uint32_t per = sub ? (noc / nsched ? noc / nsched : 1u) : noc;
+  const bool wrap = sub && noc < nsched;
+  constexpr uint64_t kUnits = (1ull << U_COUNT) - 1;
+  const auto reg = P::template lanes<int32_t>((int)noc, [&](int f) -> int32_t {
+    if (!(freem >> f & 1u)) return -1;
+    uint64_t pg = pend;
+    uint32_t gm = ~0u;
+    if (wrap) {
+      pg = 0;
+      for (uint32_t sc = (uint32_t)f; sc < nsched; sc += noc) pg |= pend & (kUnits << (sc * U_COUNT));
+      gm = 1u << f;
+    } else if (sub) {
+      const uint32_t g = (uint32_t)f / per;
+      pg = g < nsched ? pend & (kUnits << (g * U_COUNT)) : 0ull;
+      gm = ((1u << per) - 1u) << (g * per);
+    }
+    for (uint32_t k = (uint32_t)popc64(freem & gm & ((1u << f) - 1u)); k && pg; --k) pg &= pg - 1;
+    return pg ? (int32_t)ffs64(pg) : -1;
+  });
+  const uint64_t takes = P::ballot((int)noc, [&](int f) -> bool { return reg.self(f) >= 0; });
+  if (!takes) return;
+  const auto meta = P::template gather<uint64_t>(takes, s.idoc_meta, [&](int f) -> int { return reg.self(f); });
+  P::each_m(takes, [&](int f) {
+    const int bit = reg.self(f);
+    const uint32_t sc = (uint32_t)bit / U_COUNT, u = (uint32_t)bit % U_COUNT;
+    const uint64_t m = meta.self(f);
+    const TInst rin = s.idoc_inst[bit];
+    const uint32_t rw = (uint32_t)(m & 0xffu);
+    s.oc_inst[f] = rin;
+    uint64_t bk = 0;
+    uint32_t nread = 0;
+    for (int j = 0; j < 5; ++j) {
+      const uint8_t r = rin.src[j];
+      const uint32_t bank = r ? reg_bank(c, sc, rw, r - 1u) : 0xffu;
+      bk |= (uint64_t)(bank & 0xffu) << (8 * j);
+      nread += r ? 1u : 0u;
+    }
+    bk |= (uint64_t)nread << 40 | (uint64_t)rin.dst[0] << 48 | (uint64_t)rin.dst[1] << 56;
+    s.oc_banks[f] = bk;
+    s.oc_info[f] = (uint64_t)rw | (uint64_t)sc << 8 | (uint64_t)u << 16 | ((m >> 8) & 0xffull) << 24 |
+                   (uint64_t)rin.lat << 32 | (uint64_t)rin.ii << 48;
+    s.oc_age[f] = (uint32_t)(m >> 32);
+  });
+  const uint64_t reads =
+      P::ballot_m(takes, [&](int f) -> bool { return (((uint64_t)s.oc_banks[f] >> 40) & 0xffu) != 0; });
+  const uint64_t moved = P::vor((int)noc, [&](int f) -> uint64_t {
+    const int32_t b = reg.self(f);
+    return b >= 0 ? 1ull << b : 0ull;
+  });
+  s.oc_mask = ocm | (uint32_t)takes;
+  if (reads) s.oc_read_mask |= (uint32_t)reads;
+  s.idoc_mask = pend & ~moved;
+  P::sync();
 }
 
 template <class P, class S>
```

After: 287,500. 4.5% lower.
